# josebeo2016/SCL-Deepfake-audio-detection

Hardware: AMD Instinct MI355X
Metric: train-step utterances/sec (64000-sample clips) (higher is better)
Workload: dtype bf16

## Files before the change

include/scl_hip.h:

```cpp
#ifndef SCL_HIP_H
#define SCL_HIP_H
#include <stdint.h>
#include <stddef.h>

#ifdef __cplusplus
extern "C" {
#endif

#define SCL_OK            0
#define SCL_EINVAL       -1
#define SCL_ELAUNCH      -2
#define SCL_EUNSUPPORTED -3

int         scl_version(void);
const char* scl_last_error(void);

int scl_stream_wait_stream(void* waiter, void* signaler);

#define SCL_KID_GEMM 0
#define SCL_KID_GEMM_F32 2
#define SCL_KID_AUG  1
#define SCL_KID_MAX  8
int scl_build_flags(void);
int scl_prof_enable(int kid, int on);
int scl_prof_reserve(int kid, int n_pairs);
int scl_prof_read(int kid, int64_t* n_launches, double* total_ms, double* total_flops);
int scl_prof_read_launches(int kid, int cap, float* ms, int32_t* meta8, int64_t* n_launches);

typedef struct SclOperand {
    const void* ptr;
    int64_t bs1, bs2;
    int64_t rbstride;
    int64_t cout;
    int32_t rpb;
    int32_t ld;
    int32_t cin;
    int32_t _pad;
} SclOperand;

#define SCL_GEMM_A_T      0x00000001
#define SCL_GEMM_B_T      0x00000002
#define SCL_GEMM_C_F32    0x00000004
#define SCL_GEMM_C2_F32   0x00000008
#define SCL_GEMM_R_F32    0x00000010
#define SCL_GEMM_HAS_BIAS 0x00000020
#define SCL_GEMM_HAS_C2   0x00000040
#define SCL_GEMM_DROPOUT  0x00000080
#define SCL_GEMM_NO_DMA   0x00100000
#define SCL_GEMM_NO_BIG   0x00200000
#define SCL_GEMM_FORCE_BIG 0x04000000
#define SCL_GEMM_NO_P8    0x00400000
#define SCL_GEMM_FORCE_P8 0x00800000
#define SCL_GEMM_NO_W8    0x01000000
#define SCL_GEMM_F32X3    0x20000000
#define SCL_GEMM_FORCE_W8 0x02000000
#define SCL_GEMM_FORCE_X2 0x08000000
#define SCL_GEMM_NO_X2    0x10000000
#define SCL_GEMM_AB_F32   0x40000000
#define SCL_GEMM_C_SPLIT3 0x80000000u
#define SCL_GEMM_STAMPS   0x20000000
#define SCL_GEMM_ACT_SHIFT   8
#define SCL_GEMM_RMODE_SHIFT 12
#define SCL_GEMM_RACT_SHIFT  16

typedef struct SclGemmDesc {
    SclOperand A, B;
    void*        C;
    void*        C2;
    const void*  R;
    const float* bias;
    int64_t c_bs1, c_bs2;
    int64_t c_rbstride;
    int64_t c_split_stride;
    int64_t bias_bs2;
    int32_t c_rpb, ldc;
    int32_t M, N, K;
    int32_t nb1, nb2, splitk;
    int32_t flags;
    float    alpha;
    float    drop_p;
    uint32_t drop_seed;
    int32_t  _pad;
    float*   colsum_part;
} SclGemmDesc;

int scl_gemm_bf16(const SclGemmDesc* desc, void* stream);
int scl_gemm_bf16_group_ok(const SclGemmDesc* descs, int n);
int scl_gemm_bf16_group(const SclGemmDesc* descs, int n, void* stream);
int scl_gemm_bf16_group_tiles(const SclGemmDesc* desc);
int scl_gemm_bf16_group_part(const SclGemmDesc* descs, const int32_t* tile0, const int32_t* ntile, int n, void* stream);

int scl_gemm_uses_wide_tiles(const SclGemmDesc* desc);
int scl_gemm_colsum_rows(const SclGemmDesc* desc);

int scl_posconv_supported(int T, int K, int G, int Cg);
int scl_posconv_wgrad_supported(int T, int K, int G, int Cg);
int scl_posconv_wgrad(const void* dypad, int dy_row0, const void* xpad, float* dw, int B, int T, int K, int G, int Cg, void* stream);
int scl_posconv_mfma(const void* xpad, const void* w, float* C, const float* bias, void* c2, const float* R, int B, int T, int K, int G,
                     int Cg, int fwd, void* stream);

int scl_debug_gemm_stamps(unsigned long long* out, int nblocks);
long long scl_debug_gemm_persistent_launches(void);

int scl_gemm_splitk_finish(const SclGemmDesc* desc, const float* slabs, int nslabs, int64_t stride, void* stream);

int scl_reduce_slabs_f32(const float* slabs, float* out, int64_t n, int nslabs, int64_t stride, void* stream);
#define SCL_SLAB_MAX_JOBS 8
typedef struct SclSlabJob {
    const float* slabs;
    float*       out;
    int64_t      n, stride;
    int32_t      nslabs, _pad;
} SclSlabJob;
int scl_reduce_slabs_multi(const SclSlabJob* jobs, int njobs, void* stream);

int scl_bn_nslabs(int N);
int scl_bn_fwd(const float* x, int N, int C, const float* gamma, const float* beta, float* running_mean, float* running_var,
               long long* num_batches_tracked, int training, float momentum, float eps, int act, float* part, float* mean,
               float* rstd, float* y, void* y2, int y2_bf16, int m_W, int m_HW, int64_t m_bs, int64_t m_rs, int64_t m_cs,
               int64_t m_base, void* stream);
int scl_bn_bwd(const float* dy, const float* y, const float* x, const float* mean, const float* rstd, const float* gamma, int N, int C,
               int act, int training, float* part, float* sums, float* dgamma, float* dbeta, float* dx, int accumulate, void* stream);
int scl_pad_nhwc_f32(const float* src, int64_t rows, int C, void* dst, int dst_bf16, int m_W, int m_HW, int64_t m_bs, int64_t m_rs,
                     int64_t m_cs, int64_t m_base, void* stream);
int scl_conv_pack_weights(const float* w, float* fwd, float* bwd, int Co, int Ci, int kh, int kw, int Cp, int Cop, void* stream);
int scl_conv_wgrad_finish(const float* slabs, float* grad, int nslab, int Co, int Ci, int kh, int kw, int Cp, int accumulate, void* stream);
int scl_maxpool3_fwd(const float* x, int64_t xs_h, int64_t xs_w, int64_t xs_b, int H, int W, int B, float* y, int* idx, void* stream);
int scl_maxpool3_bwd(const float* dy, const int* idx, int H, int W, int B, float* dx, int64_t xs_h, int64_t xs_w, int64_t xs_b, void* stream);
int scl_avgpool_fwd(const float* x, int B, int R, int C, float* y, void* stream);
int scl_avgpool_bwd(const float* dy, int B, int R, int C, float* dx, void* stream);

int scl_layernorm_fwd(const void* x, int x_f32, const float* gamma, const float* beta, void* y_bf16, float* y_f32,
                      float* mean, float* rstd, int M, int C, int64_t ldx, int64_t ldy, float eps, int act, void* stream);
int scl_layernorm_bwd_nparts(int M);
int scl_layernorm_bwd(const void* dy, int dy_f32, const void* x, int x_f32, const float* mean, const float* rstd,
                      const float* gamma, const float* beta, const float* dres, float* dx_f32, void* dx_bf16,
                      float* part, int M, int C, int64_t ldx, int64_t lddy, int64_t lddx, int act, int sum_dres, int out_rpb,
                      int64_t out_rbstride, int64_t out_off, uint32_t din_seed, float din_p, uint32_t dout_seed, float dout_p, void* stream);
int scl_colreduce_f32(const float* part, float* out, int nparts, int C, int64_t pstride, int accumulate, void* stream);
#define SCL_COLREDUCE_SEGMENTS 8
#define SCL_COLSUM_MAX_GROUPS 128
#define SCL_REDUCE_MAX_JOBS 8
typedef struct SclReduceJob {
    const float* part;
    float*       out;
    float*       out2;
    int64_t      pstride;
    int32_t      nparts, C, split, _pad;
} SclReduceJob;
int scl_colreduce_multi(const SclReduceJob* jobs, int njobs, void* stream);
int scl_colreduce_seg_f32(const float* part, float* out, int nparts, int C, int64_t pstride, int accumulate, float* scratch, int* counters,
                          float* out2, int split, void* stream);
int scl_colsum_nparts(int M);
int scl_colsum_reduce_nparts(int M, int N);
int scl_colsum(const void* x, int x_f32, float* part, int M, int N, int64_t ld, void* stream);
int scl_colsum_reduce(const void* x, int x_f32, float* part, int* counters, float* out, int M, int N, int64_t ld, void* stream);

int scl_cast_f32_bf16(const float* src, void* dst, int64_t n, void* stream);
int scl_split3_f32_bf16(const float* x, int64_t rows, int K, int64_t ldx, void* out, int order, void* stream);
int scl_add_f32(const float* a, const float* b, float* out, void* out_bf16, int64_t n, void* stream);
int scl_pad_rows_bf16(const void* src, int src_f32, void* dst, const void* pre, int ract, int B, int T, int C,
                      int rows_out, int pad_before, void* stream);
int scl_col2im_bf16(const void* dcol, void* dz, int B, int Tin, int Tout, int C, int k, int s, void* stream);
int scl_conv_weight_pack(const float* w, void* wk, void* wd, int Co, int Ci, int k, int stride, void* stream);
int scl_conv_weight_unpack_grad(const float* dwk, float* dw, int Co, int Ci, int k, void* stream);
int scl_posconv_weight_pack(const float* v, const float* g, float* norm, void* wf, void* wd, int E, int Cg, int K, void* stream);
int scl_posconv_weight_bwd(const float* dwf, const float* v, const float* g, const float* norm, float* sdot_ws,
                           float* dv, float* dg, int E, int Cg, int K, void* stream);
int scl_dropout_f32(const float* x, float* y_f32, void* y_bf16, int64_t n, uint32_t seed, float p, void* stream);
int scl_dropout_rows(const void* x, void* y, int64_t R, int T, int ld, int is_f32, uint32_t seed, float p, void* stream);
int scl_meanpool_fwd(const void* h, float* emb, int B, int T, int C, void* stream);
int scl_meanpool_bwd(const float* demb, const void* pre, void* dpre, int B, int T, int C, int ract, float drop_p,
                     uint32_t seed, void* stream);
int scl_meanpool_fwd_f32(const float* h, float* emb, int B, int T, int C, void* stream);
int scl_meanpool_bwd_f32(const float* demb, const float* pre, float* dpre, int B, int T, int C, int ract, float drop_p,
                         uint32_t seed, void* stream);
int scl_utt_head_fwd(const float* emb, const float* W, const float* bias, float* logp, int B, int C, int NC, void* stream);
int scl_utt_head_bwd(const float* dlogp, const float* logp, const float* emb, const float* W, const float* demb_in,
                     float* demb, float* dW, float* db, float* ws, int B, int C, int NC, void* stream);

int scl_softmax_fwd(const float* S, void* P, int64_t R, int T, int ldS, int Tp, void* stream);
int scl_softmax_bwd(const void* P, const float* dP, void* dS, int64_t R, int T, int lddP, int Tp, void* stream);
int scl_softmax_fwd_f32(const float* S, float* P, int64_t R, int T, int ldS, int Tp, void* stream);
int scl_softmax_fwd_f32_long(const float* S, float* P, int64_t R, int T, int ldS, int Tp, void* stream);
int scl_attn_fwd(const void* qkv, void* ctx, float* lse, int B, int T, int H, int D, float scale, float drop_p, uint32_t drop_seed,
                 void* stream);
int scl_attn_fwd_fp8(const void* qkv, void* ctx, float* lse, int B, int T, int H, int D, float scale, void* stream);
int scl_attn_bwd(const void* qkv, const void* ctx, const void* dctx, const float* lse, void* dqkv, float* bias_part, int B, int T,
                 int H, int D, float scale, float drop_p, uint32_t drop_seed, void* stream);
// ... 195 lines not shown
```

scl-deepfake-audio-detection_amd/csrc/elementwise.hip:

```cpp
#include "common.h"

namespace {

__global__ void cast_f32_bf16_kernel(const float* __restrict__ src, bf16_t* __restrict__ dst, int64_t n) {
    const int64_t i0 = ((int64_t)blockIdx.x * blockDim.x + threadIdx.x) * 8;
    const int64_t step = (int64_t)gridDim.x * blockDim.x * 8;
    for (int64_t i = i0; i < n; i += step) {
        if (i + 8 <= n) {
            const float4 a = *reinterpret_cast<const float4*>(src + i);
            const float4 b = *reinterpret_cast<const float4*>(src + i + 4);
            uint4 u;
            u.x = pack_bf2(a.x, a.y); u.y = pack_bf2(a.z, a.w); u.z = pack_bf2(b.x, b.y); u.w = pack_bf2(b.z, b.w);
            *reinterpret_cast<uint4*>(dst + i) = u;
        } else {
            for (int64_t j = i; j < n; ++j) dst[j] = f2bf(src[j]);
        }
    }
}

__global__ void split3_kernel(const float* __restrict__ x, bf16_t* __restrict__ out, int64_t rows, int K, int64_t ldx, int order) {
    const int kv = K >> 3;
    const int64_t total = rows * kv;
    const int64_t step = (int64_t)gridDim.x * blockDim.x;
    for (int64_t i = (int64_t)blockIdx.x * blockDim.x + threadIdx.x; i < total; i += step) {
// ... 66 lines not shown
    const int c8n = C / 8;
    const int64_t total = (int64_t)B * Tin * c8n;
    const int64_t i0 = (int64_t)blockIdx.x * blockDim.x + threadIdx.x;
    const int64_t step = (int64_t)gridDim.x * blockDim.x;
    for (int64_t i = i0; i < total; i += step) {
        const int c = (int)(i % c8n) * 8;
        const int64_t br = i / c8n;
        const int r = (int)(br % Tin), b = (int)(br / Tin);
        float acc[8] = {0, 0, 0, 0, 0, 0, 0, 0};
        for (int j = 0; j < k; ++j) {
            const int rj = r - j;
            if (rj < 0 || (rj % s) != 0) continue;
            const int t = rj / s;
            if (t >= Tout) continue;
            const uint4 w = *reinterpret_cast<const uint4*>(dcol + (((int64_t)b * Tout + t) * k + j) * C + c);
            const uint32_t ww[4] = {w.x, w.y, w.z, w.w};
#pragma unroll
            for (int q = 0; q < 4; ++q) { acc[2 * q] += __uint_as_float(ww[q] << 16); acc[2 * q + 1] += __uint_as_float(ww[q] & 0xFFFF0000u); }
        }
        uint4 u;
        u.x = pack_bf2(acc[0], acc[1]); u.y = pack_bf2(acc[2], acc[3]); u.z = pack_bf2(acc[4], acc[5]); u.w = pack_bf2(acc[6], acc[7]);
        *reinterpret_cast<uint4*>(dz + ((int64_t)b * Tin + r) * C + c) = u;
    }
}

__global__ void conv_w_pack_kernel(const float* __restrict__ w, bf16_t* __restrict__ wk, bf16_t* __restrict__ wd, int Co, int Ci, int k,
                                   int stride) {
    const int64_t n = (int64_t)Co * Ci * k;
    for (int64_t i = (int64_t)blockIdx.x * blockDim.x + threadIdx.x; i < n; i += (int64_t)gridDim.x * blockDim.x) {
        const int ci = (int)(i % Ci);
        const int j = (int)((i / Ci) % k);
        const int co = (int)(i / ((int64_t)Ci * k));
        const bf16_t v = f2bf(w[((int64_t)co * Ci + ci) * k + j]);
        wk[i] = v;
        if (wd) {
            const int p = j % stride, q = j / stride;
            int blk = 0;
            for (int pp = 0; pp < p; ++pp) blk += (k - pp + stride - 1) / stride;
            const int nq = (k - p + stride - 1) / stride;
            blk += nq - 1 - q;
            wd[((int64_t)blk * Co + co) * Ci + ci] = v;
        }
    }
}
__global__ void conv_w_unpack_grad_kernel(const float* __restrict__ dwk, float* __restrict__ dw, int Co, int Ci, int k) {
    const int64_t n = (int64_t)Co * Ci * k;
    for (int64_t i = (int64_t)blockIdx.x * blockDim.x + threadIdx.x; i < n; i += (int64_t)gridDim.x * blockDim.x) {
        const int j = (int)(i % k);
        const int ci = (int)((i / k) % Ci);
        const int co = (int)(i / ((int64_t)Ci * k));
        dw[i] = dwk[((int64_t)co * k + j) * Ci + ci];
    }
}

__global__ __launch_bounds__(256) void posconv_norm_part_kernel(const float* __restrict__ v, float* __restrict__ part, int nrows, int K,
                                                                int rows_per_block) {
    __shared__ float red[256];
    const int j = threadIdx.x % K, rl = threadIdx.x / K, rstep = blockDim.x / K;
    const int r0 = blockIdx.x * rows_per_block, r1 = min(nrows, r0 + rows_per_block);
    float s = 0.f;
    for (int r = r0 + rl; r < r1; r += rstep) { const float t = v[(int64_t)r * K + j]; s += t * t; }
    red[threadIdx.x] = s;
    __syncthreads();
    if (threadIdx.x < K) {
        float t = 0.f;
        for (int q = 0; q < rstep; ++q) t += red[q * K + threadIdx.x];
        part[(int64_t)blockIdx.x * K + threadIdx.x] = t;
    }
}
__global__ __launch_bounds__(1024) void posconv_vec_finish_kernel(const float* __restrict__ part, float* __restrict__ out, int nparts, int K,
                                                                   int do_sqrt) {
    __shared__ float red[1024];
    const int j = threadIdx.x % K, seg = threadIdx.x / K, nseg = blockDim.x / K;
    float s = 0.f;
    for (int p = seg; p < nparts; p += nseg) s += part[(int64_t)p * K + j];
    red[threadIdx.x] = s;
    __syncthreads();
    if (threadIdx.x < K) {
        float t = 0.f;
        for (int q = 0; q < nseg; ++q) t += red[q * K + threadIdx.x];
        out[threadIdx.x] = do_sqrt ? sqrtf(t) : t;
    }
}
__global__ void posconv_pack_kernel(const float* __restrict__ v, const float* __restrict__ g, const float* __restrict__ norm,
                                    bf16_t* __restrict__ wf, bf16_t* __restrict__ wd, int E, int Cg, int K) {
    const int64_t n = (int64_t)E * Cg * K;
    for (int64_t i = (int64_t)blockIdx.x * blockDim.x + threadIdx.x; i < n; i += (int64_t)gridDim.x * blockDim.x) {
        const int j = (int)(i % K);
        const int ci = (int)((i / K) % Cg);
        const int cot = (int)(i / ((int64_t)Cg * K));
        const int grp = cot / Cg, co = cot % Cg;
        const bf16_t val = f2bf(g[j] * v[i] / norm[j]);
        wf[(((int64_t)grp * Cg + co) * K + j) * Cg + ci] = val;
        wd[(((int64_t)grp * Cg + ci) * K + (K - 1 - j)) * Cg + co] = val;
    }
}
__global__ __launch_bounds__(256) void posconv_wbwd_dot_part_kernel(const float* __restrict__ dwf, const float* __restrict__ v,
                                                                    float* __restrict__ part, int Cg, int K) {
    extern __shared__ float sm[];
    float* vl = sm;
    float* dl = sm + Cg * K;
    float* red = dl + K * (Cg + 1);
    const int cot = blockIdx.x;
    const float* vb = v + (int64_t)cot * Cg * K;
    const float* db = dwf + (int64_t)cot * K * Cg;
    for (int i = threadIdx.x; i < Cg * K; i += blockDim.x) {
        vl[i] = vb[i];
        dl[(i / Cg) * (Cg + 1) + (i % Cg)] = db[i];
    }
    __syncthreads();
    const int j = threadIdx.x % K, h = threadIdx.x / K, nh = blockDim.x / K;
    float s = 0.f;
    for (int ci = h; ci < Cg; ci += nh) s += dl[j * (Cg + 1) + ci] * vl[ci * K + j];
    red[threadIdx.x] = s;
    __syncthreads();
    if (threadIdx.x < K) {
        float t = 0.f;
        for (int q = 0; q < nh; ++q) t += red[q * K + threadIdx.x];
        part[(int64_t)cot * K + threadIdx.x] = t;
    }
}
__global__ void posconv_wbwd_apply_kernel(const float* __restrict__ dwf, const float* __restrict__ v, const float* __restrict__ g,
                                          const float* __restrict__ norm, const float* __restrict__ sdot,
                                          float* __restrict__ dv, float* __restrict__ dg, int E, int Cg, int K) {
    const int64_t n = (int64_t)E * Cg * K;
    for (int64_t i = (int64_t)blockIdx.x * blockDim.x + threadIdx.x; i < n; i += (int64_t)gridDim.x * blockDim.x) {
        const int j = (int)(i % K);
        const int ci = (int)((i / K) % Cg);
        const int cot = (int)(i / ((int64_t)Cg * K));
        const int grp = cot / Cg, co = cot % Cg;
        const float dw = dwf[(((int64_t)grp * Cg + co) * K + j) * Cg + ci];
        const float nj = norm[j];
        dv[i] = g[j] / nj * dw - g[j] * sdot[j] / (nj * nj * nj) * v[i];
        if (i < K) dg[i] = sdot[i] / norm[i];
    }
}

__device__ __forceinline__ float ld_act(const bf16_t* p, int64_t i) { return bf2f(p[i]); }
__device__ __forceinline__ float ld_act(const float* p, int64_t i) { return p[i]; }
__device__ __forceinline__ void st_act(bf16_t* p, int64_t i, float v) { p[i] = f2bf(v); }
__device__ __forceinline__ void st_act(float* p, int64_t i, float v) { p[i] = v; }
template <typename TA>
__global__ __launch_bounds__(512) void meanpool_fwd_kernel(const TA* __restrict__ h, float* __restrict__ emb, int T, int C) {
    __shared__ float red[4][128];
    const int b = blockIdx.x, g = threadIdx.x >> 7, l = threadIdx.x & 127;
    for (int c0 = 0; c0 < C; c0 += 128) {
        const int c = c0 + l;
        float s = 0.f;
        if (c < C)
            for (int t = g; t < T; t += 4) s += ld_act(h, ((int64_t)b * T + t) * C + c);
        red[g][l] = s;
        __syncthreads();
        if (g == 0 && c < C) emb[(int64_t)b * C + c] = (((red[0][l] + red[1][l]) + red[2][l]) + red[3][l]) / (float)T;
        __syncthreads();
    }
}
template <typename TA>
__global__ void meanpool_bwd_kernel(const float* __restrict__ demb, const TA* __restrict__ pre, TA* __restrict__ dpre,
                                    int B, int T, int C, int ract, float drop_p, uint32_t seed) {
    const int64_t n = (int64_t)B * T * C;
    for (int64_t i = (int64_t)blockIdx.x * blockDim.x + threadIdx.x; i < n; i += (int64_t)gridDim.x * blockDim.x) {
        const int c = (int)(i % C);
        const int b = (int)(i / ((int64_t)T * C));
        float v = demb[(int64_t)b * C + c] / (float)T;
        if (drop_p > 0.f) v *= dropout_scale(seed, (uint64_t)i, drop_p);
        v *= act_grad_f(ract, ld_act(pre, i));
        st_act(dpre, i, v);
    }
}
__global__ void utt_head_fwd_kernel(const float* __restrict__ emb, const float* __restrict__ W, const float* __restrict__ bias,
                                    float* __restrict__ logp, int B, int C, int NC) {
    const int b = blockIdx.x * (blockDim.x >> 6) + (threadIdx.x >> 6);
    const int lane = threadIdx.x & 63;
    if (b >= B) return;
    float lg[8];
    float mx = -INFINITY;
    for (int k = 0; k < NC; ++k) {
        float s = 0.f;
        for (int c = lane; c < C; c += 64) s += emb[(int64_t)b * C + c] * W[(int64_t)k * C + c];
        s = wave_sum(s) + bias[k];
        lg[k] = s;
        mx = fmaxf(mx, s);
    }
    float se = 0.f;
    for (int k = 0; k < NC; ++k) se += expf(lg[k] - mx);
    const float lse = mx + logf(se);
    if (lane == 0) for (int k = 0; k < NC; ++k) logp[(int64_t)b * NC + k] = lg[k] - lse;
}
__global__ void utt_head_bwd_kernel(const float* __restrict__ dlogp, const float* __restrict__ logp, const float* __restrict__ emb,
                                    const float* __restrict__ W, const float* __restrict__ demb_in, float* __restrict__ demb,
                                    float* __restrict__ dW, float* __restrict__ db, float* __restrict__ dlogits_ws, int B,
                                    int C, int NC) {
    for (int i = threadIdx.x; i < B; i += blockDim.x) {
        float s = 0.f;
        for (int k = 0; k < NC; ++k) s += dlogp[i * NC + k];
        for (int k = 0; k < NC; ++k) dlogits_ws[i * NC + k] = dlogp[i * NC + k] - expf(logp[i * NC + k]) * s;
    }
    __syncthreads();
    for (int i = threadIdx.x; i < B * C; i += blockDim.x) {
        const int b = i / C, c = i % C;
        float s = demb_in ? demb_in[i] : 0.f;
        for (int k = 0; k < NC; ++k) s += dlogits_ws[b * NC + k] * W[(int64_t)k * C + c];
        demb[i] = s;
    }
    for (int i = threadIdx.x; i < NC * C; i += blockDim.x) {
        const int k = i / C, c = i % C;
        float s = 0.f;
        for (int b = 0; b < B; ++b) s += dlogits_ws[b * NC + k] * emb[(int64_t)b * C + c];
        dW[i] = s;
    }
    for (int k = threadIdx.x; k < NC; k += blockDim.x) {
        float s = 0.f;
        for (int b = 0; b < B; ++b) s += dlogits_ws[b * NC + k];
        db[k] = s;
    }
}

__global__ void add_f32_kernel(const float* __restrict__ a, const float* __restrict__ b, float* __restrict__ out,
                               bf16_t* __restrict__ out_bf, int64_t n) {
    for (int64_t i = (int64_t)blockIdx.x * blockDim.x + threadIdx.x; i < n; i += (int64_t)gridDim.x * blockDim.x) {
        const float v = a[i] + (b ? b[i] : 0.f);
        if (out) out[i] = v;
        if (out_bf) out_bf[i] = f2bf(v);
    }
}

inline int grid_for(int64_t n, int per_thread = 1) {
    int64_t b = (n / per_thread + 255) / 256;
    if (b > 4096) b = 4096;
    if (b < 1) b = 1;
    return (int)b;
}

}

extern "C" int scl_cast_f32_bf16(const float* src, void* dst, int64_t n, void* stream) {
    SCL_REQUIRE(src && dst && n > 0 && ((uintptr_t)src & 15) == 0 && ((uintptr_t)dst & 15) == 0, "cast: bad args");
    hipLaunchKernelGGL(cast_f32_bf16_kernel, dim3(grid_for(n, 8)), dim3(256), 0, (hipStream_t)stream, src, (bf16_t*)dst, n);
    return scl_check_launch("scl_cast_f32_bf16");
}

extern "C" int scl_split3_f32_bf16(const float* x, int64_t rows, int K, int64_t ldx, void* out, int order, void* stream) {
    SCL_REQUIRE(x && out && rows > 0 && K >= 8 && (K & 7) == 0 && ldx >= K && (ldx & 3) == 0 && (order == 0 || order == 1), "split3: bad args (K a multiple of 8)");
    SCL_REQUIRE(((uintptr_t)x & 15) == 0 && ((uintptr_t)out & 15) == 0, "split3: operands must be 16-byte aligned");
    hipLaunchKernelGGL(split3_kernel, dim3(grid_for(rows * (K >> 3))), dim3(256), 0, (hipStream_t)stream, x, (bf16_t*)out, rows, K, ldx, order);
    return scl_check_launch("scl_split3_f32_bf16");
}

extern "C" int scl_pad_rows_bf16(const void* src, int src_f32, void* dst, const void* pre, int ract, int B, int T, int C,
                                 int rows_out, int pad_before, void* stream) {
    SCL_REQUIRE(src && dst && B > 0 && T > 0 && C > 0 && (C & 7) == 0 && rows_out >= 1, "pad_rows: bad args");
    const int64_t total = (int64_t)B * rows_out * (C / 8);
    hipStream_t s = (hipStream_t)stream;
    if (src_f32) hipLaunchKernelGGL((pad_rows_kernel<true>), dim3(grid_for(total)), dim3(256), 0, s, src, (bf16_t*)dst, (const bf16_t*)pre, B, T, C, rows_out, pad_before, ract);
    else hipLaunchKernelGGL((pad_rows_kernel<false>), dim3(grid_for(total)), dim3(256), 0, s, src, (bf16_t*)dst, (const bf16_t*)pre, B, T, C, rows_out, pad_before, ract);
    return scl_check_launch("scl_pad_rows_bf16");
}

extern "C" int scl_col2im_bf16(const void* dcol, void* dz, int B, int Tin, int Tout, int C, int k, int s, void* stream) {
    SCL_REQUIRE(dcol && dz && B > 0 && Tin > 0 && Tout > 0 && (C & 7) == 0 && k >= 1 && s >= 1, "col2im: bad args");
    const int64_t total = (int64_t)B * Tin * (C / 8);
    hipLaunchKernelGGL(col2im_kernel, dim3(grid_for(total)), dim3(256), 0, (hipStream_t)stream, (const bf16_t*)dcol, (bf16_t*)dz, B, Tin, Tout, C, k, s);
    return scl_check_launch("scl_col2im_bf16");
}

extern "C" int scl_conv_weight_pack(const float* w, void* wk, void* wd, int Co, int Ci, int k, int stride, void* stream) {
    SCL_REQUIRE(w && wk && Co > 0 && Ci > 0 && k > 0 && stride >= 1, "conv_weight_pack: bad args");
    hipLaunchKernelGGL(conv_w_pack_kernel, dim3(grid_for((int64_t)Co * Ci * k)), dim3(256), 0, (hipStream_t)stream, w, (bf16_t*)wk,
                       (bf16_t*)wd, Co, Ci, k, stride);
    return scl_check_launch("scl_conv_weight_pack");
}
extern "C" int scl_conv_weight_unpack_grad(const float* dwk, float* dw, int Co, int Ci, int k, void* stream) {
    SCL_REQUIRE(dwk && dw && Co > 0 && Ci > 0 && k > 0, "conv_weight_unpack_grad: bad args");
    hipLaunchKernelGGL(conv_w_unpack_grad_kernel, dim3(grid_for((int64_t)Co * Ci * k)), dim3(256), 0, (hipStream_t)stream, dwk, dw, Co, Ci, k);
    return scl_check_launch("scl_conv_weight_unpack_grad");
}

extern "C" int scl_posconv_weight_pack(const float* v, const float* g, float* norm, void* wf, void* wd, int E, int Cg, int K, void* stream) {
    SCL_REQUIRE(v && g && norm && wf && wd && E > 0 && Cg > 0 && K > 0 && E % Cg == 0, "posconv_weight_pack: bad args");
    hipStream_t s = (hipStream_t)stream;
    {
        SCL_REQUIRE(K <= 256 && 256 % K == 0 && E * Cg >= 2, "posconv_weight_pack: need K | 256");
        const int nrows = E * Cg;
        int nb = nrows / 2 < 256 ? nrows / 2 : 256;
        const int rpb = (nrows + nb - 1) / nb;
        float* part = reinterpret_cast<float*>(wd);
        hipLaunchKernelGGL(posconv_norm_part_kernel, dim3((nrows + rpb - 1) / rpb), dim3(256), 0, s, v, part, nrows, K, rpb);
        hipLaunchKernelGGL(posconv_vec_finish_kernel, dim3(1), dim3(1024 / K * K), 0, s, part, norm, (nrows + rpb - 1) / rpb, K, 1);
    }
    hipLaunchKernelGGL(posconv_pack_kernel, dim3(grid_for((int64_t)E * Cg * K)), dim3(256), 0, s, v, g, norm, (bf16_t*)wf, (bf16_t*)wd, E, Cg, K);
    return scl_check_launch("scl_posconv_weight_pack");
}
extern "C" int scl_posconv_weight_bwd(const float* dwf, const float* v, const float* g, const float* norm, float* sdot_ws,
                                      float* dv, float* dg, int E, int Cg, int K, void* stream) {
    SCL_REQUIRE(dwf && v && g && norm && sdot_ws && dv && dg, "posconv_weight_bwd: null pointer");
    hipStream_t s = (hipStream_t)stream;
    {
        SCL_REQUIRE(K <= 256 && 256 % K == 0, "posconv_weight_bwd: need K | 256");
        float* part = sdot_ws + K;
        const size_t lds = (size_t)(Cg * K + K * (Cg + 1) + 256) * sizeof(float);
        static bool attr_set = false;
        if (!attr_set) {
            hipFuncSetAttribute((const void*)posconv_wbwd_dot_part_kernel, hipFuncAttributeMaxDynamicSharedMemorySize, 160 * 1024);
            attr_set = true;
        }
        SCL_REQUIRE(lds <= 160 * 1024, "posconv_weight_bwd: Cg*K too large for the LDS tile");
        hipLaunchKernelGGL(posconv_wbwd_dot_part_kernel, dim3(E), dim3(256), lds, s, dwf, v, part, Cg, K);
        hipLaunchKernelGGL(posconv_vec_finish_kernel, dim3(1), dim3(1024 / K * K), 0, s, part, sdot_ws, E, K, 0);
    }
    hipLaunchKernelGGL(posconv_wbwd_apply_kernel, dim3(grid_for((int64_t)E * Cg * K)), dim3(256), 0, s, dwf, v, g, norm, sdot_ws, dv, dg, E, Cg, K);
    return scl_check_launch("scl_posconv_weight_bwd");
}

extern "C" int scl_meanpool_fwd(const void* h, float* emb, int B, int T, int C, void* stream) {
    SCL_REQUIRE(h && emb && B > 0 && T > 0 && C > 0, "meanpool_fwd: bad args");
    hipLaunchKernelGGL(meanpool_fwd_kernel<bf16_t>, dim3(B), dim3(512), 0, (hipStream_t)stream, (const bf16_t*)h, emb, T, C);
    return scl_check_launch("scl_meanpool_fwd");
}
extern "C" int scl_meanpool_fwd_f32(const float* h, float* emb, int B, int T, int C, void* stream) {
    SCL_REQUIRE(h && emb && B > 0 && T > 0 && C > 0, "meanpool_fwd_f32: bad args");
    hipLaunchKernelGGL(meanpool_fwd_kernel<float>, dim3(B), dim3(512), 0, (hipStream_t)stream, h, emb, T, C);
    return scl_check_launch("scl_meanpool_fwd_f32");
}
extern "C" int scl_meanpool_bwd(const float* demb, const void* pre, void* dpre, int B, int T, int C, int ract, float drop_p,
                                uint32_t seed, void* stream) {
    SCL_REQUIRE(demb && pre && dpre && B > 0 && T > 0 && C > 0, "meanpool_bwd: bad args");
    hipLaunchKernelGGL(meanpool_bwd_kernel<bf16_t>, dim3(grid_for((int64_t)B * T * C)), dim3(256), 0, (hipStream_t)stream, demb, (const bf16_t*)pre, (bf16_t*)dpre, B, T, C, ract, drop_p, seed);
    return scl_check_launch("scl_meanpool_bwd");
}
extern "C" int scl_meanpool_bwd_f32(const float* demb, const float* pre, float* dpre, int B, int T, int C, int ract, float drop_p,
                                    uint32_t seed, void* stream) {
    SCL_REQUIRE(demb && pre && dpre && B > 0 && T > 0 && C > 0, "meanpool_bwd_f32: bad args");
    hipLaunchKernelGGL(meanpool_bwd_kernel<float>, dim3(grid_for((int64_t)B * T * C)), dim3(256), 0, (hipStream_t)stream, demb, pre, dpre, B, T, C, ract, drop_p, seed);
    return scl_check_launch("scl_meanpool_bwd_f32");
}
extern "C" int scl_utt_head_fwd(const float* emb, const float* W, const float* bias, float* logp, int B, int C, int NC, void* stream) {
    SCL_REQUIRE(emb && W && bias && logp && B > 0 && C > 0 && NC >= 1 && NC <= 8, "utt_head_fwd: bad args");
    hipLaunchKernelGGL(utt_head_fwd_kernel, dim3((B + 3) / 4), dim3(256), 0, (hipStream_t)stream, emb, W, bias, logp, B, C, NC);
    return scl_check_launch("scl_utt_head_fwd");
}
extern "C" int scl_utt_head_bwd(const float* dlogp, const float* logp, const float* emb, const float* W, const float* demb_in,
                                float* demb, float* dW, float* db, float* ws, int B, int C, int NC, void* stream) {
    SCL_REQUIRE(dlogp && logp && emb && W && demb && dW && db && ws && B > 0 && NC <= 8, "utt_head_bwd: bad args");
    hipLaunchKernelGGL(utt_head_bwd_kernel, dim3(1), dim3(256), 0, (hipStream_t)stream, dlogp, logp, emb, W, demb_in, demb, dW, db, ws, B, C, NC);
    return scl_check_launch("scl_utt_head_bwd");
}
__global__ void dropout_f32_kernel(const float* __restrict__ x, float* __restrict__ y, bf16_t* __restrict__ y_bf, int64_t n, uint32_t seed, float p) {
    for (int64_t i = (int64_t)blockIdx.x * blockDim.x + threadIdx.x; i < n; i += (int64_t)gridDim.x * blockDim.x) {
        const float v = x[i] * dropout_scale(seed, (uint64_t)i, p);
        if (y) y[i] = v;
        if (y_bf) y_bf[i] = f2bf(v);
    }
}
extern "C" int scl_dropout_f32(const float* x, float* y_f32, void* y_bf16, int64_t n, uint32_t seed, float p, void* stream) {
    SCL_REQUIRE(x && (y_f32 || y_bf16) && n > 0 && p >= 0.f && p < 1.f, "dropout_f32: bad args");
    hipLaunchKernelGGL(dropout_f32_kernel, dim3(grid_for(n)), dim3(256), 0, (hipStream_t)stream, x, y_f32, (bf16_t*)y_bf16, n, seed, p);
    return scl_check_launch("scl_dropout_f32");
}
template <typename TX>
__global__ void dropout_rows_kernel(const TX* __restrict__ x, TX* __restrict__ y, int64_t R, int T, int ld, uint32_t seed, float p) {
    const int64_t n = R * ld;
    for (int64_t i = (int64_t)blockIdx.x * blockDim.x + threadIdx.x; i < n; i += (int64_t)gridDim.x * blockDim.x) {
        const int64_t r = i / ld;
        const int j = (int)(i - r * ld);
        float v = 0.f;
        if (j < T) {
            if constexpr (sizeof(TX) == 2) v = bf2f(x[i]); else v = x[i];
            v *= dropout_scale(seed, (uint64_t)(r * T + j), p);
        }
        if constexpr (sizeof(TX) == 2) y[i] = f2bf(v); else y[i] = v;
    }
}
extern "C" int scl_dropout_rows(const void* x, void* y, int64_t R, int T, int ld, int is_f32, uint32_t seed, float p, void* stream) {
    SCL_REQUIRE(x && y && R > 0 && T > 0 && ld >= T && p >= 0.f && p < 1.f, "dropout_rows: bad args");
    if (is_f32) hipLaunchKernelGGL(dropout_rows_kernel<float>, dim3(grid_for(R * ld)), dim3(256), 0, (hipStream_t)stream, (const float*)x, (float*)y, R, T, ld, seed, p);
    else hipLaunchKernelGGL(dropout_rows_kernel<bf16_t>, dim3(grid_for(R * ld)), dim3(256), 0, (hipStream_t)stream, (const bf16_t*)x, (bf16_t*)y, R, T, ld, seed, p);
    return scl_check_launch("scl_dropout_rows");
}
extern "C" int scl_add_f32(const float* a, const float* b, float* out, void* out_bf16, int64_t n, void* stream) {
    SCL_REQUIRE(a && (out || out_bf16) && n > 0, "add_f32: bad args");
    hipLaunchKernelGGL(add_f32_kernel, dim3(grid_for(n)), dim3(256), 0, (hipStream_t)stream, a, b, out, (bf16_t*)out_bf16, n);
    return scl_check_launch("scl_add_f32");
}
```

scl-deepfake-audio-detection_amd/csrc/gemm.hip:

```cpp
#include "gemm_common.h"

using namespace sclg;

namespace {

constexpr int BM = 128, BN = 128;

struct StageK {
    __amdgpu_buffer_rsrc_t rsrc;
    unsigned rowoff[4];
    unsigned lds_off[4];
    int kcur, kend;

    __device__ __forceinline__ void init(const OpK& o, const char* base, int row0, int rowlimit, int kbegin, int kend_, int tid) {
        rsrc = make_rsrc(base);
        const int c = tid & 7;
#pragma unroll
        for (int i = 0; i < 4; ++i) {
            const int row = (tid >> 3) + 32 * i;
            const int r = row0 + row;
            rowoff[i] = r < rowlimit ? row_off(o, (unsigned)r) : OOB;
            lds_off[i] = (unsigned)(row * 128 + ((c ^ ((row >> 1) & 7)) << 4));
        }
        kcur = kbegin + 8 * c; kend = kend_;
// ... 549 lines not shown

    f32x4 acc[2][4][4];
#pragma unroll
    for (int h = 0; h < 2; ++h)
#pragma unroll
        for (int i = 0; i < 4; ++i)
#pragma unroll
            for (int j = 0; j < 4; ++j) acc[h][i][j] = f32x4{0.f, 0.f, 0.f, 0.f};

#define P8_ISSUE_A(BUF) { la0.issue(d.A, (BUF), wave); la1.issue(d.A, (BUF) + TILE_BYTES, wave); la0.advance(); la1.advance(); }
#define P8_ISSUE_B(BUF) { lb0.issue(d.B, (BUF) + 2 * TILE_BYTES, wave); lb1.issue(d.B, (BUF) + 3 * TILE_BYTES, wave); lb0.advance(); lb1.advance(); }

    P8_ISSUE_A(smem) P8_ISSUE_B(smem) P8_ISSUE_B(smem + P8_BUF)
    asm volatile("s_waitcnt vmcnt(4)" ::: "memory");
    __builtin_amdgcn_s_barrier();
    if (wr == 1) __builtin_amdgcn_s_barrier();

    bf16x8 fa[4][2], fb0[2][2], fb1[2][2];
    for (int kt = 0; kt < nk; ++kt) {
        char* buf = smem + (kt & 1) * P8_BUF;
        char* obuf = smem + ((kt & 1) ^ 1) * P8_BUF;
        const char* tA = buf + wr * TILE_BYTES;
        const char* tB = buf + (2 + (wc >> 1)) * TILE_BYTES;
        const int nb = (wc & 1) * 4;
#pragma unroll
        for (int ks = 0; ks < 2; ++ks) {
#pragma unroll
            for (int j = 0; j < 2; ++j) fb0[j][ks] = BT ? frag_t_raw(tB, nb + j, ks, lane) : frag_k(tB, nb + j, ks, lane);
        }
        __builtin_amdgcn_sched_barrier(0);
#pragma unroll
        for (int ks = 0; ks < 2; ++ks) {
#pragma unroll
            for (int i = 0; i < 4; ++i) fa[i][ks] = AT ? frag_t_raw(tA, i, ks, lane) : frag_k(tA, i, ks, lane);
        }
        P8_ISSUE_A(obuf)
        P8_PHASE(0, 0, fb0)
#pragma unroll
        for (int ks = 0; ks < 2; ++ks) {
#pragma unroll
            for (int j = 0; j < 2; ++j) fb1[j][ks] = BT ? frag_t_raw(tB, nb + 2 + j, ks, lane) : frag_k(tB, nb + 2 + j, ks, lane);
        }
        P8_PHASE(0, 1, fb1)
#pragma unroll
        for (int ks = 0; ks < 2; ++ks) {
#pragma unroll
            for (int i = 0; i < 4; ++i) fa[i][ks] = AT ? frag_t_raw(tA, 4 + i, ks, lane) : frag_k(tA, 4 + i, ks, lane);
        }
        P8_PHASE(1, 1, fb1)
        asm volatile("s_waitcnt vmcnt(0)" ::: "memory");
        P8_ISSUE_B(buf)
        P8_PHASE(1, 0, fb0)
    }
    if (wr == 0) __builtin_amdgcn_s_barrier();
    asm volatile("s_waitcnt vmcnt(0)" ::: "memory");
    gemm_epilogue(d, acc[0], m0 + wr * 128, n0 + wc * 64, z1, z2, ksplit, lane, 0, 0);
    gemm_epilogue(d, acc[1], m0 + wr * 128 + 64, n0 + wc * 64, z1, z2, ksplit, lane, 0, 0);
}
#undef P8_PHASE
#undef P8_ISSUE_A
#undef P8_ISSUE_B

#endif

__global__ void scl_reduce_slabs_kernel(const float* __restrict__ slabs, float* __restrict__ out, int64_t n,
                                        int nslabs, int64_t stride) {
    const int64_t i0 = ((int64_t)blockIdx.x * blockDim.x + threadIdx.x) * 4;
    const int64_t step = (int64_t)gridDim.x * blockDim.x * 4;
    for (int64_t i = i0; i < n; i += step) {
        if (i + 4 <= n) {
            float4 s = *reinterpret_cast<const float4*>(slabs + i);
            for (int k = 1; k < nslabs; ++k) {
                const float4 t = *reinterpret_cast<const float4*>(slabs + k * stride + i);
                s.x += t.x; s.y += t.y; s.z += t.z; s.w += t.w;
            }
            *reinterpret_cast<float4*>(out + i) = s;
        } else {
            for (int64_t j = i; j < n; ++j) {
                float s = slabs[j];
                for (int k = 1; k < nslabs; ++k) s += slabs[k * stride + j];
                out[j] = s;
            }
        }
    }
}

}

namespace sclg {
void make_magic(unsigned dv, unsigned* magic, unsigned* shift) {
    unsigned l = 0;
    while ((1ull << l) < dv) ++l;
    *shift = l;
    *magic = (unsigned)((((1ull << l) - dv) << 32) / dv + 1);
}

bool fill_operand(const SclOperand& o, const char* name, long long rows, long long contig, OpK* k, int esz) {
    const int vec = 16 / esz;
    if (!o.ptr || ((uintptr_t)o.ptr & 15)) { scl_set_error("gemm: %s ptr null or not 16B aligned", name); return false; }
    if (o.rpb < 1 || o.cin < vec) { scl_set_error("gemm: %s rpb/cin invalid", name); return false; }
    if ((o.ld % vec) || (o.rbstride % vec) || (o.cout % vec) || (o.bs1 % vec) || (o.bs2 % vec) || (o.cin != 0x7fffffff && (o.cin % vec))) {
        scl_set_error("gemm: %s strides must be multiples of %d elements", name, vec); return false;
    }
    const long long rq = (rows - 1) / o.rpb, rr = o.rpb == 0x7fffffff ? rows - 1 : (long long)o.rpb - 1;
    const long long cq = o.cin == 0x7fffffff ? 0 : (contig - 1) / o.cin;
    const long long cr = o.cin == 0x7fffffff ? contig - 1 : (long long)o.cin - 1;
    const long long maxoff = rq * o.rbstride + (rr < rows - 1 ? rr : rows - 1) * (long long)o.ld + cq * o.cout + cr + vec;
    if (maxoff < 0 || maxoff * esz >= (1ll << 32) - 32 || rows >= (1ll << 31)) {
        scl_set_error("gemm: %s extent exceeds 32-bit byte offsets (%lld elements)", name, maxoff); return false;
    }
    k->ptr = o.ptr; k->bs1 = o.bs1 * esz; k->bs2 = o.bs2 * esz;
    k->rb_bytes = (unsigned)(o.rbstride * esz); k->ld_bytes = (unsigned)o.ld * (unsigned)esz; k->cout_bytes = (unsigned)(o.cout * esz);
    k->rpb = (unsigned)o.rpb; make_magic((unsigned)o.rpb, &k->rpb_magic, &k->rpb_shift);
    k->cin = (unsigned)o.cin; make_magic((unsigned)o.cin, &k->cin_magic, &k->cin_mshift);
    k->esz_shift = esz == 4 ? 2u : 1u;
    return true;
}
}

namespace {

bool gemm_pick_w8(const GemmK& k, bool at, bool bt, const SclGemmDesc& d, long long zdim, W8Plan* plan) {
    const int w8_env = 1;
    if (d.flags & (SCL_GEMM_NO_W8 | SCL_GEMM_FORCE_P8 | SCL_GEMM_FORCE_BIG | SCL_GEMM_NO_DMA)) return false;
    const bool a_whole = at ? (d.M % 8 == 0) : (d.K % 8 == 0);
    const bool b_whole = bt ? (d.N % 8 == 0) : (d.K % 8 == 0);
    static const int ncu_env = [] { const char* e = getenv("SCL_GEMM_CUS"); const int v = e ? atoi(e) : 256; return v >= 32 && v <= 256 ? v : 256; }();
    if (!a_whole || !b_whole || !scl_gemm_w8_plan(k, at, bt, d, zdim, ncu_env, plan)) return false;
    const long long need = at ? 128 : 160;
    return (d.flags & SCL_GEMM_FORCE_W8) || (w8_env && d.N >= 192 && plan->tiles * zdim >= need);
}

#ifdef SCL_EXPERIMENTS
bool gemm_pick_x2(const GemmK& k, bool at, bool bt, const SclGemmDesc& d, long long zdim, W8Plan* plan) {
    static const int x2_env = [] { const char* e = getenv("SCL_GEMM_X2"); return e ? atoi(e) : 0; }();
    if (d.flags & (SCL_GEMM_NO_X2 | SCL_GEMM_FORCE_W8 | SCL_GEMM_FORCE_P8 | SCL_GEMM_FORCE_BIG | SCL_GEMM_NO_DMA)) return false;
    if (!(d.flags & SCL_GEMM_FORCE_X2) && x2_env == 0) return false;
    const bool a_whole = at ? (d.M % 8 == 0) : (d.K % 8 == 0);
    const bool b_whole = bt ? (d.N % 8 == 0) : (d.K % 8 == 0);
    static const int ncu_env = [] { const char* e = getenv("SCL_GEMM_CUS"); const int v = e ? atoi(e) : 256; return v >= 32 && v <= 256 ? v : 256; }();
    if (!a_whole || !b_whole || !scl_gemm_x2_plan(k, at, bt, d, zdim, ncu_env, plan)) return false;
    if ((d.flags & SCL_GEMM_FORCE_X2) || x2_env == 2) return true;
    return !at && d.N >= 128 && plan->tiles * zdim >= 248;
}

#else
bool gemm_pick_x2(const GemmK&, bool, bool, const SclGemmDesc&, long long, W8Plan*) { return false; }
#endif
}

extern "C" int scl_gemm_uses_wide_tiles(const SclGemmDesc* dp) {
    if (!dp || dp->M <= 0 || dp->N <= 0 || dp->K <= 0 || dp->nb1 < 1 || dp->nb2 < 1 || dp->splitk < 1) return 0;
    GemmK k; W8Plan plan;
    const bool at = dp->flags & SCL_GEMM_A_T, bt = dp->flags & SCL_GEMM_B_T;
    const long long zdim = (long long)dp->nb1 * dp->nb2 * dp->splitk;
    if (gemm_pick_x2(k, at, bt, *dp, zdim, &plan)) return 3;
    return gemm_pick_w8(k, at, bt, *dp, zdim, &plan) ? (plan.variant == 2 ? 4 : 1 + plan.variant) : 0;
}

static int gemm_colsum_rows(const SclGemmDesc& d) {
    if (d.M <= 0 || d.N <= 0 || d.K <= 0 || d.nb1 != 1 || d.nb2 != 1 || d.splitk != 1 || (d.N & 7) || (d.ldc & 7) || (d.flags & SCL_GEMM_AB_F32)) return 0;
    GemmK k; W8Plan plan;
    const bool at = d.flags & SCL_GEMM_A_T, bt = d.flags & SCL_GEMM_B_T;
    const bool a_whole = at ? (d.M % 8 == 0) : (d.K % 8 == 0), b_whole = bt ? (d.N % 8 == 0) : (d.K % 8 == 0);
    SclGemmDesc dq = d;
    if (!dq.colsum_part) dq.colsum_part = reinterpret_cast<float*>(16);
// ... 243 lines not shown
    float v[4] = {0.f, 0.f, 0.f, 0.f};
    const bool full = col + 4 <= d.N && !(d.N & 3) && !(stride & 3);
    for (int s = 0; s < nslabs; ++s, p += stride) {
        if (full) {
            const float4 t = *reinterpret_cast<const float4*>(p);
            v[0] += t.x; v[1] += t.y; v[2] += t.z; v[3] += t.w;
        } else {
            for (int i = 0; i < 4; ++i) if (col + i < d.N) v[i] += p[i];
        }
    }
    const unsigned q = udiv_magic((unsigned)row, d.c_magic, d.c_shift);
    const long long off = (long long)q * d.c_rbstride + (long long)((unsigned)row - q * d.c_rpb) * d.ldc + col;
    const float* bias = (flags & SCL_GEMM_HAS_BIAS) ? d.bias : nullptr;
    if (full && d.vec_ok) {
        const bool c_f32 = flags & SCL_GEMM_C_F32, c2_f32 = flags & SCL_GEMM_C2_F32, r_f32 = flags & SCL_GEMM_R_F32;
        const int act = (flags >> SCL_GEMM_ACT_SHIFT) & 0xF, rmode = (flags >> SCL_GEMM_RMODE_SHIFT) & 0xF, ract = (flags >> SCL_GEMM_RACT_SHIFT) & 0xF;
        if (bias) {
            const float4 bb = *reinterpret_cast<const float4*>(bias + col);
            v[0] += bb.x; v[1] += bb.y; v[2] += bb.z; v[3] += bb.w;
        }
        float c2v[4] = {v[0], v[1], v[2], v[3]};
        if (act == 5) { gelu_both_f(v[0], v[0], c2v[0]); gelu_both_f(v[1], v[1], c2v[1]); gelu_both_f(v[2], v[2], c2v[2]); gelu_both_f(v[3], v[3], c2v[3]); }
        if (flags & SCL_GEMM_HAS_C2) {
            if (c2_f32) *reinterpret_cast<float4*>(reinterpret_cast<float*>(d.C2) + off) = make_float4(c2v[0], c2v[1], c2v[2], c2v[3]);
            else *reinterpret_cast<uint2*>(reinterpret_cast<bf16_t*>(d.C2) + off) = make_uint2(pack_bf2(c2v[0], c2v[1]), pack_bf2(c2v[2], c2v[3]));
        }
        if (act && act != 5) { v[0] = act_f(act, v[0]); v[1] = act_f(act, v[1]); v[2] = act_f(act, v[2]); v[3] = act_f(act, v[3]); }
        float r[4] = {0.f, 0.f, 0.f, 0.f};
        if (rmode) {
            if (r_f32) {
                const float4 t = *reinterpret_cast<const float4*>(reinterpret_cast<const float*>(d.R) + off);
                r[0] = t.x; r[1] = t.y; r[2] = t.z; r[3] = t.w;
            } else {
                const uint2 t = *reinterpret_cast<const uint2*>(reinterpret_cast<const bf16_t*>(d.R) + off);
                r[0] = __uint_as_float(t.x << 16); r[1] = __uint_as_float(t.x & 0xFFFF0000u);
                r[2] = __uint_as_float(t.y << 16); r[3] = __uint_as_float(t.y & 0xFFFF0000u);
            }
        }
#pragma unroll
        for (int i = 0; i < 4; ++i) {
            if (rmode == 2) v[i] *= act_grad_f(ract, r[i]);
            if (flags & SCL_GEMM_DROPOUT) v[i] *= dropout_scale(d.drop_seed, (uint64_t)(off + i), d.drop_p);
            if (rmode == 1) v[i] += r[i];
        }
        if (c_f32) *reinterpret_cast<float4*>(reinterpret_cast<float*>(d.C) + off) = make_float4(v[0], v[1], v[2], v[3]);
        else *reinterpret_cast<uint2*>(reinterpret_cast<bf16_t*>(d.C) + off) = make_uint2(pack_bf2(v[0], v[1]), pack_bf2(v[2], v[3]));
    } else {
        const EpiArgs ea = {d.C, d.C2, d.R, d.N, d.flags, d.drop_seed, d.drop_p};
        for (int i = 0; i < 4; ++i) epi_scalar(ea, v[i], off + i, col + i, bias);
    }
}

extern "C" int scl_gemm_splitk_finish(const SclGemmDesc* dp, const float* slabs, int nslabs, int64_t stride, void* stream) {
    SCL_REQUIRE(dp && slabs && nslabs >= 1 && stride >= 0, "gemm finish: bad args");
    const SclGemmDesc& d = *dp;
    SCL_REQUIRE(d.M > 0 && d.N > 0 && d.nb1 == 1 && d.nb2 == 1, "gemm finish: one un-batched [M, N] problem");
    SCL_REQUIRE(d.C && d.c_rpb >= 1, "gemm finish: C null or c_rpb < 1");
    const int rmode = (d.flags >> SCL_GEMM_RMODE_SHIFT) & 0xF;
    SCL_REQUIRE(rmode == 0 || d.R, "gemm finish: RMODE set but R is null");
    SCL_REQUIRE(!(d.flags & SCL_GEMM_HAS_C2) || d.C2, "gemm finish: HAS_C2 set but C2 is null");
    SCL_REQUIRE(!(d.flags & SCL_GEMM_HAS_BIAS) || d.bias, "gemm finish: HAS_BIAS set but bias is null");
    SCL_REQUIRE(((uintptr_t)slabs & 15) == 0, "gemm finish: slabs must be 16-byte aligned");
    GemmK k;
    k.C = d.C; k.C2 = d.C2; k.R = d.R; k.bias = d.bias; k.colsum = nullptr;
    k.c_bs1 = 0; k.c_bs2 = 0; k.c_rbstride = d.c_rbstride; k.c_split_stride = 0; k.bias_bs2 = 0;
    k.c_rpb = (unsigned)d.c_rpb; make_magic((unsigned)d.c_rpb, &k.c_magic, &k.c_shift);
    k.ldc = d.ldc; k.M = d.M; k.N = d.N; k.K = d.K; k.nb2 = 1; k.splitk = 1; k.flags = d.flags;
    k.alpha = 1.0f; k.drop_p = d.drop_p; k.drop_seed = d.drop_seed; k.group_m = 8; k.tile_m = 0; k.debug = 0;
    auto al = [](const void* p, int bytes) { return p == nullptr || ((uintptr_t)p & (bytes - 1)) == 0; };
    k.vec_ok = !(d.ldc & 3) && !(d.c_rbstride & 3) && al(d.C, (d.flags & SCL_GEMM_C_F32) ? 16 : 8) && al(d.C2, (d.flags & SCL_GEMM_C2_F32) ? 16 : 8) &&
               al(d.R, (d.flags & SCL_GEMM_R_F32) ? 16 : 8) && al(d.bias, 16);
    const long long n = (long long)d.M * ((d.N + 3) / 4);
    hipLaunchKernelGGL(scl_gemm_finish_kernel, dim3((unsigned)((n + 255) / 256)), dim3(256), 0, (hipStream_t)stream, k, slabs, nslabs, (long long)stride);
    return scl_check_launch("scl_gemm_splitk_finish");
}

extern "C" int scl_reduce_slabs_f32(const float* slabs, float* out, int64_t n, int nslabs, int64_t stride, void* stream) {
    SCL_REQUIRE(slabs && out && n > 0 && nslabs >= 1, "reduce_slabs: bad args");
    SCL_REQUIRE(((uintptr_t)slabs & 15) == 0 && ((uintptr_t)out & 15) == 0 && (stride & 3) == 0, "reduce_slabs: alignment");
    int blocks = (int)((n / 4 + 255) / 256); if (blocks > 2048) blocks = 2048; if (blocks < 1) blocks = 1;
    hipLaunchKernelGGL(scl_reduce_slabs_kernel, dim3(blocks), dim3(256), 0, (hipStream_t)stream, slabs, out, n, nslabs, stride);
    return scl_check_launch("scl_reduce_slabs_f32");
}
```

scl-deepfake-audio-detection_amd/csrc/gemm_w8.hip:

```cpp
#include "gemm_common.h"
#include "gemm_w8_epi.h"

using namespace sclg;

__device__ unsigned long long scl_gemm_stamps[4096 * 8];

namespace {

__device__ __forceinline__ void w8_stamp(const GemmK& d, int slot, int lane, int wave) {
    if ((d.flags & SCL_GEMM_STAMPS) && wave == 0 && lane == 0 && blockIdx.x < 4096 && blockIdx.z == 0) {
        scl_gemm_stamps[blockIdx.x * 8 + 2 * slot] = __builtin_amdgcn_s_memrealtime();
        scl_gemm_stamps[blockIdx.x * 8 + 2 * slot + 1] = __builtin_amdgcn_s_memtime();
    }
}

constexpr int W8_BN = 256;
constexpr int W8_OPB = 2 * TILE_BYTES;
constexpr int W8_NA = 3, W8_NB = 2;
constexpr int W8_LDS = (W8_NA + W8_NB) * W8_OPB;

struct W8K {
    __amdgpu_buffer_rsrc_t rsrc;
    unsigned voff[4];
    __device__ __forceinline__ void init(const OpK& o, const char* base, int row0, int rowlimit, int lane, int wave) {
        rsrc = make_rsrc(base);
#pragma unroll
        for (int i = 0; i < 4; ++i) {
            const int row = 8 * (wave * 4 + i) + (lane >> 3);
            const int r = row0 + row;
            const int kc = (lane & 7) ^ ((row >> 1) & 7);
            voff[i] = r < rowlimit ? row_off(o, (unsigned)r) + (unsigned)(kc << 4) : OOB;
        }
    }
    template <int I0>
    __device__ __forceinline__ void issue2(char* img, int wave, unsigned soff, bool live) const {
#pragma unroll
        for (int i = I0; i < I0 + 2; ++i) {
            const unsigned off = live ? voff[i] : OOB;
            __builtin_amdgcn_raw_ptr_buffer_load_lds(rsrc, (lds_void*)(img + (wave * 4 + i) * 1024), 16, off, soff, 0, 0);
        }
    }
    __device__ __forceinline__ void issue1(char* img, int wave, unsigned soff, bool live, int i) const {
        const unsigned off = live ? voff[i] : OOB;
        __builtin_amdgcn_raw_ptr_buffer_load_lds(rsrc, (lds_void*)(img + (wave * 4 + i) * 1024), 16, off, soff, 0, 0);
    }
    __device__ __forceinline__ static unsigned kstep(const OpK& o) { return o.cin == 64 ? o.cout_bytes : 128u; }
    __device__ __forceinline__ void rows(const OpK&, int, int, int) {}
    __device__ __forceinline__ void set_batched(bool) {}
    __device__ __forceinline__ unsigned step(const OpK& o) const { return kstep(o); }
};
struct W8T {
    __amdgpu_buffer_rsrc_t rsrc;
    unsigned voff[4];
    int col0_, collimit_;
    bool batched;
    __device__ __forceinline__ void set_batched(bool b) { batched = b; }
    __device__ __forceinline__ void init(const OpK& o, const char* base, int col0, int collimit, int lane, int wave) {
        rsrc = make_rsrc(base);
        col0_ = col0; collimit_ = collimit;
        const int s16 = lane & 15;
#pragma unroll
        for (int i = 0; i < 4; ++i) {
            const int p = wave * 4 + i;
            const int kr = 4 * (p & 15) + (lane >> 4);
            const int sw = (kr & 3) | (((kr >> 3) & 1) << 2);
            const int col = col0 + (p >> 4) * 128 + 8 * ((((s16 >> 1) ^ sw) << 1) | (s16 & 1));
            voff[i] = col < collimit ? (unsigned)kr * o.ld_bytes + col_off(o, (unsigned)col) : OOB;
        }
    }
    __device__ __forceinline__ void rows(const OpK& o, int krow, int lane, int wave) {
        if (!batched) return;
        const int s16 = lane & 15;
#pragma unroll
        for (int i = 0; i < 4; ++i) {
            const int p = wave * 4 + i;
            const int kr = 4 * (p & 15) + (lane >> 4);
            const int sw = (kr & 3) | (((kr >> 3) & 1) << 2);
            const int col = col0_ + (p >> 4) * 128 + 8 * ((((s16 >> 1) ^ sw) << 1) | (s16 & 1));
            voff[i] = col < collimit_ ? row_off(o, (unsigned)(krow + kr)) + col_off(o, (unsigned)col) : OOB;
        }
    }
    template <int I0>
    __device__ __forceinline__ void issue2(char* img, int wave, unsigned soff, bool live) const {
#pragma unroll
        for (int i = I0; i < I0 + 2; ++i) {
            const unsigned off = live ? voff[i] : OOB;
            __builtin_amdgcn_raw_ptr_buffer_load_lds(rsrc, (lds_void*)(img + (wave * 4 + i) * 1024), 16, off, soff, 0, 0);
        }
    }
    __device__ __forceinline__ void issue1(char* img, int wave, unsigned soff, bool live, int i) const {
        const unsigned off = live ? voff[i] : OOB;
        __builtin_amdgcn_raw_ptr_buffer_load_lds(rsrc, (lds_void*)(img + (wave * 4 + i) * 1024), 16, off, soff, 0, 0);
    }
    __device__ __forceinline__ static unsigned kstep(const OpK& o) { return 64u * o.ld_bytes; }
    __device__ __forceinline__ unsigned step(const OpK& o) const { return batched ? 0u : kstep(o); }
};
template <bool T> struct W8Sel { typedef W8K type; };
template <> struct W8Sel<true> { typedef W8T type; };

template <bool T>
__device__ __forceinline__ bf16x8 w8_frag(const char* img, int gb, int ks, int lane) {
    if (T) return frag_t_raw(img + (gb >> 3) * TILE_BYTES, gb & 7, ks, lane);
    return frag_k(img, gb, ks, lane);
}

#define W8_MFMA_PHASE(MH, NH, FBSEL, NI)                                                                   \
    asm volatile("s_waitcnt lgkmcnt(0)" ::: "memory");                                                     \
    __builtin_amdgcn_sched_barrier(0);                                                                     \
    __builtin_amdgcn_s_barrier();                                                                          \
    __builtin_amdgcn_sched_barrier(0);                                                                     \
    __builtin_amdgcn_s_setprio(1);                                                                         \
    _Pragma("unroll") for (int ks = 0; ks < 2; ++ks)                                                       \
        _Pragma("unroll") for (int i = 0; i < (NI); ++i)                                                   \
            _Pragma("unroll") for (int j = 0; j < 2; ++j)                                                  \
                acc[MH][i][2 * (NH) + j] = __builtin_amdgcn_mfma_f32_16x16x32_bf16(FBSEL[j][ks], fa[i][ks], acc[MH][i][2 * (NH) + j], 0, 0, 0); \
    __builtin_amdgcn_s_setprio(0);                                                                         \
    __builtin_amdgcn_sched_barrier(0);                                                                     \
    __builtin_amdgcn_s_barrier();

template <bool AT, bool BT, int NH>
__device__ __forceinline__ void w8_body(const GemmK& d, char* smem, typename W8Sel<AT>::type& la, typename W8Sel<BT>::type& lb,
                                        int nk, unsigned soffA, unsigned soffB, int ab, int m0, int n0, int mlimit,
                                        int z1, int z2, int ksplit, int lane, int wave, int wc, int krow0) {
    const unsigned stepA = la.step(d.A), stepB = lb.step(d.B);
    f32x4 acc[2][4][4];
#pragma unroll
    for (int h = 0; h < 2; ++h)
#pragma unroll
        for (int i = 0; i < 4; ++i)
#pragma unroll
            for (int j = 0; j < 4; ++j) acc[h][i][j] = f32x4{0.f, 0.f, 0.f, 0.f};

    bf16x8 fa[4][2], fb0[2][2], fb1[2][2];
    const int nbk = wc * 4;
    char* const bimg = smem + W8_NA * W8_OPB;
    char *a_cur = smem, *a_nxt = smem + W8_OPB, *a_fill = smem + 2 * W8_OPB;
    for (int kt = 0; kt < nk; ++kt) {
        const char* tA = a_cur;
        char* tB = bimg + (kt & 1) * W8_OPB;
#ifdef W8_FAKE_AB
        const bool live2 = false;
#else
        const bool live2 = kt + 2 < nk;
#endif
        soffA += stepA; soffB += stepB;
#pragma unroll
        for (int ks = 0; ks < 2; ++ks) {
#pragma unroll
            for (int j = 0; j < 2; ++j) fb0[j][ks] = w8_frag<BT>(tB, nbk + j, ks, lane);
        }
        __builtin_amdgcn_sched_barrier(0);
#pragma unroll
        for (int ks = 0; ks < 2; ++ks) {
#pragma unroll
            for (int i = 0; i < 4; ++i) fa[i][ks] = w8_frag<AT>(tA, ab + i, ks, lane);
        }
        la.rows(d.A, krow0 + (kt + 2) * BK, lane, wave);
        la.template issue2<0>(a_fill, wave, soffA, live2);
        W8_MFMA_PHASE(0, 0, fb0, 4)
#pragma unroll
        for (int ks = 0; ks < 2; ++ks) {
#pragma unroll
            for (int j = 0; j < 2; ++j) fb1[j][ks] = w8_frag<BT>(tB, nbk + 2 + j, ks, lane);
        }
        la.template issue2<2>(a_fill, wave, soffA, live2);
        W8_MFMA_PHASE(0, 1, fb1, 4)
#pragma unroll
        for (int ks = 0; ks < 2; ++ks) {
#pragma unroll
            for (int i = 0; i < NH; ++i) fa[i][ks] = w8_frag<AT>(tA, ab + 4 + i, ks, lane);
        }
        lb.rows(d.B, krow0 + (kt + 2) * BK, lane, wave);
        lb.template issue2<0>(tB, wave, soffB, live2);
        W8_MFMA_PHASE(1, 1, fb1, NH)
        lb.template issue2<2>(tB, wave, soffB, live2);
        asm volatile("s_waitcnt vmcnt(8)" ::: "memory");
        W8_MFMA_PHASE(1, 0, fb0, NH)
        char* t = a_cur; a_cur = a_nxt; a_nxt = a_fill; a_fill = t;
    }
    if ((wave >> 2) == 0) __builtin_amdgcn_s_barrier();
    asm volatile("s_waitcnt vmcnt(0)" ::: "memory");
    __builtin_amdgcn_s_barrier();
    w8_stamp(d, 2, lane, wave);
    {
        const long long cbase = z1 * d.c_bs1 + z2 * d.c_bs2 + (long long)ksplit * d.c_split_stride;
        const float* bias = (d.flags & SCL_GEMM_HAS_BIAS) ? d.bias + z2 * d.bias_bs2 : nullptr;
        char* wlds = smem + wave * 16384;
        char* wextra = smem + 8 * 16384 + wave * 4096;
        float* cs0 = d.colsum ? d.colsum + ((long long)(m0 / d.tile_m) * 4 + (wave >> 2) * 2) * d.N : nullptr;
        w8_epilogue_pass<4, 0>(d, acc[0], 4, wlds, wextra, m0 + ab * 16, n0 + wc * 64, mlimit, cbase, bias, lane, cs0);
        w8_epilogue_pass<4, 0>(d, acc[1], NH, wlds, wextra, m0 + (ab + 4) * 16, n0 + wc * 64, mlimit, cbase, bias, lane, cs0 ? cs0 + d.N : nullptr);
    }
    if (d.flags & SCL_GEMM_STAMPS) {
        asm volatile("s_waitcnt vmcnt(0)" ::: "memory");
        w8_stamp(d, 3, lane, wave);
    }
}

template <bool AT, bool BT, int RB0, int RB1>
__global__ __launch_bounds__(512, 2) void scl_gemm_w8_kernel(const GemmK d) {
    extern __shared__ __attribute__((aligned(16))) char smem[];
    const int tid = threadIdx.x, lane = tid & 63;
    const int wave = __builtin_amdgcn_readfirstlane(tid >> 6);
    const int wr = wave >> 2, wc = wave & 3;
    w8_stamp(d, 0, lane, wave);
    const int tiles_m = (d.M + d.tile_m - 1) / d.tile_m, tiles_n = (d.N + W8_BN - 1) / W8_BN;
    int tm, tn;
    tile_coords(blockIdx.x, gridDim.x, tiles_m, tiles_n, tm, tn, d.group_m);
    const int m0 = tm * d.tile_m, n0 = tn * W8_BN;
    const int mlimit = min(d.M, m0 + d.tile_m);
    int z = blockIdx.z;
    const int ksplit = __builtin_amdgcn_readfirstlane(z % d.splitk); z /= d.splitk;
    const int z1 = __builtin_amdgcn_readfirstlane(z / d.nb2), z2 = z - z1 * d.nb2;
    const int nk_total = d.K / BK;
    const int nk_per = __builtin_amdgcn_readfirstlane((nk_total + d.splitk - 1) / d.splitk);
    const int kt0 = ksplit * nk_per;
    const int nk = max(0, min(nk_per, nk_total - kt0));
    const char* Ab = reinterpret_cast<const char*>(d.A.ptr) + z1 * d.A.bs1 + z2 * d.A.bs2;
    const char* Bb = reinterpret_cast<const char*>(d.B.ptr) + z1 * d.B.bs1 + z2 * d.B.bs2;

    typename W8Sel<AT>::type la;
    typename W8Sel<BT>::type lb;
    la.init(d.A, Ab, m0, mlimit, lane, wave);
    lb.init(d.B, Bb, n0, d.N, lane, wave);
    la.set_batched(AT && (d.debug & 4));
    lb.set_batched(BT && (d.debug & 8));
    const unsigned stepA = la.step(d.A), stepB = lb.step(d.B);
    unsigned soffA = (unsigned)kt0 * stepA, soffB = (unsigned)kt0 * stepB;
    const int krow0 = kt0 * BK;

    la.rows(d.A, krow0, lane, wave); lb.rows(d.B, krow0, lane, wave);
    la.template issue2<0>(smem, wave, soffA, nk > 0); la.template issue2<2>(smem, wave, soffA, nk > 0);
    lb.template issue2<0>(smem + W8_NA * W8_OPB, wave, soffB, nk > 0); lb.template issue2<2>(smem + W8_NA * W8_OPB, wave, soffB, nk > 0);
    soffA += stepA; soffB += stepB;
    la.rows(d.A, krow0 + BK, lane, wave); lb.rows(d.B, krow0 + BK, lane, wave);
    la.template issue2<0>(smem + W8_OPB, wave, soffA, nk > 1); la.template issue2<2>(smem + W8_OPB, wave, soffA, nk > 1);
    lb.template issue2<0>(smem + (W8_NA + 1) * W8_OPB, wave, soffB, nk > 1); lb.template issue2<2>(smem + (W8_NA + 1) * W8_OPB, wave, soffB, nk > 1);
    asm volatile("s_waitcnt vmcnt(8)" ::: "memory");
    w8_stamp(d, 1, lane, wave);
    __builtin_amdgcn_s_barrier();
    if (wr == 1) __builtin_amdgcn_s_barrier();

    if (RB0 == RB1) {
        w8_body<AT, BT, RB0 - 4>(d, smem, la, lb, nk, soffA, soffB, wr * RB0, m0, n0, mlimit, z1, z2, ksplit, lane, wave, wc, krow0);
    } else if (wr == 0) {
        w8_body<AT, BT, RB0 - 4>(d, smem, la, lb, nk, soffA, soffB, 0, m0, n0, mlimit, z1, z2, ksplit, lane, wave, wc, krow0);
    } else {
        w8_body<AT, BT, RB1 - 4>(d, smem, la, lb, nk, soffA, soffB, RB0, m0, n0, mlimit, z1, z2, ksplit, lane, wave, wc, krow0);
    }
}

template <int OFF>
__device__ __forceinline__ bf16x8 lds_b128_raw(unsigned addr) {
    bf16x8 v;
    asm volatile("ds_read_b128 %0, %1 offset:%2" : "=v"(v) : "v"(addr), "n"(OFF) : "memory");
    return v;
}
template <bool AT, bool BT, int RBW>
struct W8SRead {
    static constexpr bool RAW = AT || BT;
    static __device__ __forceinline__ unsigned kaddr(const char* img, int gb, int ks, int lane) {
        const int row = gb * 16 + (lane & 15);
        const int c = 4 * ks + (lane >> 4);
        return (unsigned)(uintptr_t)(lds_void*)(img + row * 128 + ((c ^ ((row >> 1) & 7)) << 4));
    }
    template <int R, int REND>
    static __device__ __forceinline__ void step(bf16x8 (&FA)[RBW], bf16x8 (&FB)[4], const char* TA, const char* TB, unsigned ka, unsigned kb,
                                                int ab, int nbk, int ks, int lane) {
        if constexpr (R < REND) {
            if constexpr (R == 0 || (R > RBW)) {
                constexpr int j = R == 0 ? 0 : R - RBW;
                if constexpr (BT) FB[j] = frag_t_raw(TB + ((nbk + j) >> 3) * TILE_BYTES, (nbk + j) & 7, ks, lane);
                else if constexpr (RAW) FB[j] = lds_b128_raw<j * 2048>(kb);
                else FB[j] = frag_k(TB, nbk + j, ks, lane);
            } else {
                constexpr int i = R - 1;
                if constexpr (AT) FA[i] = frag_t_raw(TA + ((ab + i) >> 3) * TILE_BYTES, (ab + i) & 7, ks, lane);
                else if constexpr (RAW) FA[i] = lds_b128_raw<i * 2048>(ka);
                else FA[i] = frag_k(TA, ab + i, ks, lane);
            }
            if (RAW) __builtin_amdgcn_sched_barrier(0);
            step<R + 1, REND>(FA, FB, TA, TB, ka, kb, ab, nbk, ks, lane);
        }
    }
    template <int R0, int R1, bool ORDERED>
    static __device__ __forceinline__ void go(bf16x8 (&FA)[RBW], bf16x8 (&FB)[4], const char* TA, const char* TB, int ab, int nbk, int ks, int lane) {
        if constexpr (R0 < R1) {
            unsigned ka = 0, kb = 0;
            if constexpr (RAW && !AT) ka = kaddr(TA, ab, ks, lane);
            if constexpr (RAW && !BT) kb = kaddr(TB, nbk, ks, lane);
            if constexpr (ORDERED && !RAW) {
                step<R0, R0 + 1>(FA, FB, TA, TB, ka, kb, ab, nbk, ks, lane);
                __builtin_amdgcn_sched_barrier(0);
                go<R0 + 1, R1, true>(FA, FB, TA, TB, ab, nbk, ks, lane);
            } else {
                step<R0, R1>(FA, FB, TA, TB, ka, kb, ab, nbk, ks, lane);
            }
        }
    }
};

template <bool AT, bool BT, int RBW>
__device__ __forceinline__ void w8s_body(const GemmK& d, char* smem, const typename W8Sel<AT>::type& la, const typename W8Sel<BT>::type& lb,
                                         int nk, unsigned soffA, unsigned soffB, int ab, int m0, int n0, int mlimit,
                                         int z1, int z2, int ksplit, int lane, int wave, int wc) {
    const unsigned stepA = W8Sel<AT>::type::kstep(d.A), stepB = W8Sel<BT>::type::kstep(d.B);
    f32x4 acc[RBW][4];
#pragma unroll
    for (int i = 0; i < RBW; ++i)
#pragma unroll
        for (int j = 0; j < 4; ++j) acc[i][j] = f32x4{0.f, 0.f, 0.f, 0.f};
    bf16x8 fa0[RBW], fa1[RBW], fb0[4], fb1[4];
    const int nbk = wc * 4;
    char* const bimg = smem + W8_NA * W8_OPB;
    char *a_cur = smem, *a_nxt = smem + W8_OPB, *a_fill = smem + 2 * W8_OPB;
    constexpr int NRD = RBW + 4, OPA = AT ? 2 : 1, OPB = BT ? 2 : 1;
    constexpr int RQ0 = NRD < 4 ? NRD : 4, RQ1 = NRD < 8 ? NRD : 8, RQ2 = NRD;
    typedef W8SRead<AT, BT, RBW> RD;
    auto ops_upto = [](int n) constexpr { return (n > 0 ? OPB : 0) + (n > 1 ? (n - 1 < RBW ? n - 1 : RBW) * OPA : 0) + (n > RBW + 1 ? (n - RBW - 1) * OPB : 0); };
    lds_wait_upto(0);
    __builtin_amdgcn_sched_barrier(0);
    RD::template go<0, NRD, true>(fa0, fb0, a_cur, bimg, ab, nbk, 0, lane);
    for (int kt = 0; kt < nk; ++kt) {
        char* tB = bimg + (kt & 1) * W8_OPB;
        const bool live2 = kt + 2 < nk;
#ifdef W8S_FAKE_A
        const bool live2a = false;
#else
        const bool live2a = live2;
#endif
#ifdef W8S_FAKE_B
        const bool live2b = false;
#else
        const bool live2b = live2;
#endif
        soffA += stepA; soffB += stepB;
#define W8S_Q_FIRST(j, R0, R1)                                                                                               \
        RD::template go<R0, R1, false>(fa1, fb1, a_cur, tB, ab, nbk, 1, lane);                                               \
        __builtin_amdgcn_sched_barrier(0);                                                                                   \
        lds_wait_upto((3 - (j)) * OPB + ops_upto(R1));                                                                       \
        __builtin_amdgcn_sched_barrier(0);                                                                                   \
        _Pragma("unroll") for (int i = 0; i < RBW; ++i)                                                                      \
            acc[i][j] = __builtin_amdgcn_mfma_f32_16x16x32_bf16(fb0[j], fa0[i], acc[i][j], 0, 0, 0);                         \
        __builtin_amdgcn_sched_barrier(0);                                                                                   \
        la.issue1(a_fill, wave, soffA, live2a, j);                                                                           \
        __builtin_amdgcn_sched_barrier(0);
        W8S_Q_FIRST(0, 0, RQ0) W8S_Q_FIRST(1, RQ0, RQ1) W8S_Q_FIRST(2, RQ1, RQ2) W8S_Q_FIRST(3, RQ2, NRD)
#undef W8S_Q_FIRST
        lds_wait_upto(0);
        asm volatile("s_waitcnt vmcnt(4)" ::: "memory");
        __builtin_amdgcn_sched_barrier(0);
        __builtin_amdgcn_s_barrier();
        __builtin_amdgcn_sched_barrier(0);
        const char* tBn = bimg + ((kt & 1) ^ 1) * W8_OPB;
#define W8S_B_ISSUE(j) if ((j) < 2) { lb.issue1(tB, wave, soffB, live2b, 2 * (j)); lb.issue1(tB, wave, soffB, live2b, 2 * (j) + 1); }
#define W8S_Q_SECOND(j, R0, R1)                                                                                              \
        RD::template go<R0, R1, false>(fa0, fb0, a_nxt, tBn, ab, nbk, 0, lane);                                              \
        __builtin_amdgcn_sched_barrier(0);                                                                                   \
        _Pragma("unroll") for (int i = 0; i < RBW; ++i)                                                                      \
            acc[i][j] = __builtin_amdgcn_mfma_f32_16x16x32_bf16(fb1[j], fa1[i], acc[i][j], 0, 0, 0);                         \
        __builtin_amdgcn_sched_barrier(0);                                                                                   \
        W8S_B_ISSUE(j)                                                                                                       \
        __builtin_amdgcn_sched_barrier(0);
        W8S_Q_SECOND(0, 0, RQ0) W8S_Q_SECOND(1, RQ0, RQ1) W8S_Q_SECOND(2, RQ1, RQ2) W8S_Q_SECOND(3, RQ2, NRD)
#undef W8S_Q_SECOND
#undef W8S_B_ISSUE
        char* t = a_cur; a_cur = a_nxt; a_nxt = a_fill; a_fill = t;
    }
    asm volatile("s_waitcnt vmcnt(0)" ::: "memory");
    asm volatile("s_waitcnt lgkmcnt(0)" ::: "memory");
    __builtin_amdgcn_s_barrier();
    w8_stamp(d, 2, lane, wave);
    {
        const long long cbase = z1 * d.c_bs1 + z2 * d.c_bs2 + (long long)ksplit * d.c_split_stride;
        const float* bias = (d.flags & SCL_GEMM_HAS_BIAS) ? d.bias + z2 * d.bias_bs2 : nullptr;
        char* wlds = smem + wave * 16384;
        char* wextra = smem + 8 * 16384 + wave * 4096;
        float* cs0 = d.colsum ? d.colsum + ((long long)(m0 / d.tile_m) * 4 + (wave >> 2) * 2) * d.N : nullptr;
        if constexpr (RBW >= 4) {
            f32x4 (&alo)[4][4] = *reinterpret_cast<f32x4 (*)[4][4]>(&acc[0]);
            w8_epilogue_pass<4, ((RBW < 8 && !AT) ? 0x1E : 0)>(d, alo, 4, wlds, wextra, m0 + ab * 16, n0 + wc * 64, mlimit, cbase, bias, lane, cs0);
        } else {
            f32x4 lo[4][4];
#pragma unroll
            for (int i = 0; i < 4; ++i)
#pragma unroll
                for (int j = 0; j < 4; ++j) lo[i][j] = (i < RBW) ? acc[(i < RBW) ? i : 0][j] : f32x4{0.f, 0.f, 0.f, 0.f};
            w8_epilogue_pass<4, ((RBW < 8 && !AT) ? 0x1E : 0)>(d, lo, RBW, wlds, wextra, m0 + ab * 16, n0 + wc * 64, mlimit, cbase, bias, lane, cs0);
        }
        if (RBW > 4) {
            f32x4 hi[4][4];
#pragma unroll
            for (int i = 0; i < 4; ++i)
#pragma unroll
                for (int j = 0; j < 4; ++j) hi[i][j] = (4 + i < RBW) ? acc[(4 + i < RBW) ? 4 + i : 0][j] : f32x4{0.f, 0.f, 0.f, 0.f};
            w8_epilogue_pass<4, ((RBW < 8 && !AT) ? 0x1E : 0)>(d, hi, RBW - 4, wlds, wextra, m0 + (ab + 4) * 16, n0 + wc * 64, mlimit, cbase, bias, lane, cs0 ? cs0 + d.N : nullptr);
        }
    }
    if (d.flags & SCL_GEMM_STAMPS) {
        asm volatile("s_waitcnt vmcnt(0)" ::: "memory");
        w8_stamp(d, 3, lane, wave);
    }
}

template <bool AT, bool BT, int RB0, int RB1, bool SEQ = false>
__device__ __forceinline__ void w8s_tile(const GemmK& d, char* smem, const int bid, const int nblk, const int bz) {
    const int tid = threadIdx.x, lane = tid & 63;
    const int wave = __builtin_amdgcn_readfirstlane(tid >> 6);
    const int wr = wave >> 2, wc = wave & 3;
    w8_stamp(d, 0, lane, wave);
#ifdef SCL_EXPERIMENTS
    if ((d.debug >> 8) && (bid & 1) && bid < 256 && bz == 0) {
        for (int i = 0; i < (d.debug >> 8); ++i) __builtin_amdgcn_s_sleep(127);
    }
#endif
    const int tiles_m = (d.M + d.tile_m - 1) / d.tile_m, tiles_n = (d.N + W8_BN - 1) / W8_BN;
    int tm, tn;
    tile_coords<SEQ>(bid, nblk, tiles_m, tiles_n, tm, tn, d.group_m);
    const int m0 = tm * d.tile_m, n0 = tn * W8_BN;
    const int mlimit = min(d.M, m0 + d.tile_m);
    int z = bz;
    const int ksplit = __builtin_amdgcn_readfirstlane(z % d.splitk); z /= d.splitk;
    const int z1 = __builtin_amdgcn_readfirstlane(z / d.nb2), z2 = z - z1 * d.nb2;
    const int nk_total = d.K / BK;
    const int nk_per = __builtin_amdgcn_readfirstlane((nk_total + d.splitk - 1) / d.splitk);
    const int kt0 = ksplit * nk_per;
    const int nk = max(0, min(nk_per, nk_total - kt0));
    const char* Ab = reinterpret_cast<const char*>(d.A.ptr) + z1 * d.A.bs1 + z2 * d.A.bs2;
    const char* Bb = reinterpret_cast<const char*>(d.B.ptr) + z1 * d.B.bs1 + z2 * d.B.bs2;

    typename W8Sel<AT>::type la;
    typename W8Sel<BT>::type lb;
    la.init(d.A, Ab, m0, mlimit, lane, wave);
    lb.init(d.B, Bb, n0, d.N, lane, wave);
    la.set_batched(false); lb.set_batched(false);
    const unsigned stepA = W8Sel<AT>::type::kstep(d.A), stepB = W8Sel<BT>::type::kstep(d.B);
    unsigned soffA = (unsigned)kt0 * stepA, soffB = (unsigned)kt0 * stepB;
    la.template issue2<0>(smem, wave, soffA, nk > 0); la.template issue2<2>(smem, wave, soffA, nk > 0);
    lb.template issue2<0>(smem + W8_NA * W8_OPB, wave, soffB, nk > 0); lb.template issue2<2>(smem + W8_NA * W8_OPB, wave, soffB, nk > 0);
    soffA += stepA; soffB += stepB;
    la.template issue2<0>(smem + W8_OPB, wave, soffA, nk > 1); la.template issue2<2>(smem + W8_OPB, wave, soffA, nk > 1);
    lb.template issue2<0>(smem + (W8_NA + 1) * W8_OPB, wave, soffB, nk > 1); lb.template issue2<2>(smem + (W8_NA + 1) * W8_OPB, wave, soffB, nk > 1);
    asm volatile("s_waitcnt vmcnt(8)" ::: "memory");
    w8_stamp(d, 1, lane, wave);
    __builtin_amdgcn_s_barrier();
    if (RB0 == RB1) {
        w8s_body<AT, BT, RB0>(d, smem, la, lb, nk, soffA, soffB, wr * RB0, m0, n0, mlimit, z1, z2, ksplit, lane, wave, wc);
    } else if (wr == 0) {
        w8s_body<AT, BT, RB0>(d, smem, la, lb, nk, soffA, soffB, 0, m0, n0, mlimit, z1, z2, ksplit, lane, wave, wc);
    } else {
        w8s_body<AT, BT, RB1>(d, smem, la, lb, nk, soffA, soffB, RB0, m0, n0, mlimit, z1, z2, ksplit, lane, wave, wc);
    }
}

template <bool AT, bool BT, int RB0, int RB1>
__global__ __launch_bounds__(512, 2) void scl_gemm_w8s_kernel(const GemmK d) {
    extern __shared__ __attribute__((aligned(16))) char smem[];
    w8s_tile<AT, BT, RB0, RB1>(d, smem, blockIdx.x, gridDim.x, blockIdx.z);
}

struct GemmGroupK {
    GemmK k[W8_GROUP_MAX];
    int first[W8_GROUP_MAX + 1];
    int tile0[W8_GROUP_MAX];
    int ntiles[W8_GROUP_MAX];
    int n;
    int xcd_major;
};
typedef const __attribute__((address_space(4))) GemmGroupK* W8GArg;
template <bool AT, bool BT, int RB0, int RB1>
__global__ __launch_bounds__(512, 2) void scl_gemm_w8s_group_kernel(const GemmGroupK g) {
    extern __shared__ __attribute__((aligned(16))) char smem[];
    W8GArg gp = (W8GArg)__builtin_amdgcn_kernarg_segment_ptr();
    const int total = g.first[W8_GROUP_MAX];
    const int x = blockIdx.x & 7, idx = blockIdx.x >> 3, q = total >> 3, r = total & 7;
#ifdef SCL_EXPERIMENTS
    const int pos = (g.xcd_major ? ((x < r ? x * (q + 1) : r * (q + 1) + (x - r) * q) + idx) : (int)blockIdx.x);
#else
    const int pos = (x < r ? x * (q + 1) : r * (q + 1) + (x - r) * q) + idx;
#endif
    int mem = 0;
#pragma unroll
    for (int i = 1; i < W8_GROUP_MAX; ++i) mem += (i < g.n && pos >= g.first[i]) ? 1 : 0;
    mem = __builtin_amdgcn_readfirstlane(mem);
    const int t = __builtin_amdgcn_readfirstlane(pos - gp->first[mem] + gp->tile0[mem]);
#ifdef SCL_EXPERIMENTS
    if (!g.xcd_major) { w8s_tile<AT, BT, RB0, RB1, false>(*(const GemmK*)&gp->k[mem], smem, t, gp->ntiles[mem], 0); return; }
#endif
    w8s_tile<AT, BT, RB0, RB1, true>(*(const GemmK*)&gp->k[mem], smem, t, gp->ntiles[mem], 0);
}

#ifdef SCL_EXPERIMENTS
typedef const __attribute__((address_space(4))) GemmK* W8KArg;
__device__ __forceinline__ const GemmK* w8p_args(W8KArg p) {
    asm volatile("" : "+s"(p));
    return (const GemmK*)p;
}
template <bool AT, bool BT, int RBW>
__device__ __forceinline__ void w8p_body(const GemmK& d, W8KArg kp, char* smem, const char* Ab, const char* Bb, int ab, int tiles_m, int tiles_n,
                                         int lane, int wave, int wc) {
    typedef typename W8Sel<AT>::type LA;
    typedef typename W8Sel<BT>::type LB;
    const unsigned stepA = LA::kstep(d.A), stepB = LB::kstep(d.B);
    const int nk = d.K / BK;
    const int ntiles = tiles_m * tiles_n, G = gridDim.x;
    const int nbk = wc * 4;
    char* const bimg = smem + W8_NA * W8_OPB;
    char *a_cur = smem, *a_nxt = smem + W8_OPB, *a_fill = smem + 2 * W8_OPB;
    int bpar = 0;
    int v = blockIdx.x, tm, tn;
    tile_coords(v, ntiles, tiles_m, tiles_n, tm, tn, d.group_m);
    const int tile_m = d.tile_m, Mrows = d.M, group_m = d.group_m;
    int m0 = tm * tile_m, n0 = tn * W8_BN, mlimit = min(Mrows, m0 + tile_m);
    LA la;
    LB lb;
    la.init(d.A, Ab, m0, mlimit, lane, wave);
    lb.init(d.B, Bb, n0, d.N, lane, wave);
    la.set_batched(false); lb.set_batched(false);
    la.template issue2<0>(a_cur, wave, 0u, true); la.template issue2<2>(a_cur, wave, 0u, true);
    lb.template issue2<0>(bimg, wave, 0u, true); lb.template issue2<2>(bimg, wave, 0u, true);
    la.template issue2<0>(a_nxt, wave, stepA, true); la.template issue2<2>(a_nxt, wave, stepA, true);
    lb.template issue2<0>(bimg + W8_OPB, wave, stepB, true); lb.template issue2<2>(bimg + W8_OPB, wave, stepB, true);
    asm volatile("s_waitcnt vmcnt(8)" ::: "memory");
    __builtin_amdgcn_s_barrier();
#define W8S_READ(FA, FB, TA, TB, KS)                                                        \
    _Pragma("unroll") for (int j = 0; j < 4; ++j) FB[j] = w8_frag<BT>(TB, nbk + j, KS, lane); \
    _Pragma("unroll") for (int i = 0; i < RBW; ++i) FA[i] = w8_frag<AT>(TA, ab + i, KS, lane);
#define W8S_MFMA(FA, FB)                                                                    \
    _Pragma("unroll") for (int i = 0; i < RBW; ++i)                                         \
        _Pragma("unroll") for (int j = 0; j < 4; ++j)                                       \
            acc[i][j] = __builtin_amdgcn_mfma_f32_16x16x32_bf16(FB[j], FA[i], acc[i][j], 0, 0, 0);
    for (;;) {
        f32x4 acc[RBW][4];
#pragma unroll
        for (int i = 0; i < RBW; ++i)
#pragma unroll
            for (int j = 0; j < 4; ++j) acc[i][j] = f32x4{0.f, 0.f, 0.f, 0.f};
        bf16x8 fa0[RBW], fa1[RBW], fb0[4], fb1[4];
        const int vn = v + G;
        const bool has_next = vn < ntiles;
        int m0n = 0, n0n = 0, mlimn = 0;
        if (has_next) {
            tile_coords(vn, ntiles, tiles_m, tiles_n, tm, tn, group_m);
            m0n = tm * tile_m; n0n = tn * W8_BN; mlimn = min(Mrows, m0n + tile_m);
        }
        unsigned soffA = stepA, soffB = stepB;
        W8S_READ(fa0, fb0, a_cur, bimg + bpar * W8_OPB, 0)
        for (int kt = 0; kt < nk; ++kt) {
            char* tB = bimg + ((kt + bpar) & 1) * W8_OPB;
            const bool hand = kt + 2 == nk;
            const bool live2 = kt + 2 < nk || (hand && has_next);
            soffA += stepA; soffB += stepB;
            asm volatile("s_waitcnt lgkmcnt(0)" ::: "memory");
            __builtin_amdgcn_sched_barrier(0);
            W8S_READ(fa1, fb1, a_cur, tB, 1)
            __builtin_amdgcn_sched_barrier(0);
            W8S_MFMA(fa0, fb0)
            __builtin_amdgcn_sched_barrier(0);
            if (hand && has_next) {
                const GemmK* dh = w8p_args(kp);
                la.init(dh->A, reinterpret_cast<const char*>(dh->A.ptr), m0n, mlimn, lane, wave);
            }
            {
                const unsigned sa = hand ? 0u : soffA;
                la.template issue2<0>(a_fill, wave, sa, live2); la.template issue2<2>(a_fill, wave, sa, live2);
            }
            asm volatile("s_waitcnt lgkmcnt(0)" ::: "memory");
            asm volatile("s_waitcnt vmcnt(4)" ::: "memory");
            __builtin_amdgcn_sched_barrier(0);
            __builtin_amdgcn_s_barrier();
            __builtin_amdgcn_sched_barrier(0);
            if (hand && has_next) {
// ... 140 lines not shown
    const bool b_ok = bt ? (flat_rows(d.B, d.K) || (tt && d.B.rpb >= 1)) : (d.B.cin == 0x7fffffff || d.B.cin == 64 || d.B.cin >= d.K);
    if (!a_ok || !b_ok || (d.K % BK) != 0) return false;
    const long long tiles_n = (d.N + W8_BN - 1) / W8_BN;
    long long best = -1;
    const char* e43 = getenv("SCL_W8_TILE112");
    const char* epp = getenv("SCL_W8_MODE");
    const bool v43_env = !e43 || atoi(e43) != 0, pingpong_env = epp && *epp && atoi(epp) == 0;
    const bool v43_ok = v43_env && !pingpong_env && !at && zdim == 1 && !d.colsum_part && !(d.flags & SCL_GEMM_STAMPS);
    for (int v = 0; v < (v43_ok ? 3 : 2); ++v) {
        const int bm = v == 0 ? 208 : (v == 1 ? 256 : 112);
        const long long ntm = (d.M + bm - 1) / bm;
        const long long rounds = (ntm * tiles_n * zdim + ncu - 1) / ncu;
        const long long cost = rounds * (bm + W8_BN);
        if (best < 0 || cost < best) {
            best = cost;
            plan->variant = v; plan->tiles_m = (int)ntm; plan->tile_m = (int)((d.M + ntm - 1) / ntm);
            plan->tiles = ntm * tiles_n; plan->cost = cost; plan->ncu = ncu;
        }
    }
    return true;
}

bool scl_gemm_w8_group_member_ok(const GemmK& k, bool at, bool bt, const SclGemmDesc& d) {
    if (!at || !bt || d.nb1 != 1 || d.nb2 != 1 || d.splitk != 1 || (d.K % BK) != 0 || d.K / BK < 3) return false;
    if ((long long)d.A.rpb < (long long)d.K || (long long)d.B.rpb < (long long)d.K) return false;
    if ((d.M % 8) || (d.N % 8) || !k.vec_ok) return false;
    const int plain = SCL_GEMM_A_T | SCL_GEMM_B_T | SCL_GEMM_C_F32;
    return (d.flags & ~(SCL_GEMM_NO_DMA | SCL_GEMM_NO_W8)) == plain && !d.colsum_part;
}

int scl_gemm_w8_group_tiles(const GemmK& k) { return ((k.M + 255) / 256) * ((k.N + W8_BN - 1) / W8_BN); }

int scl_gemm_w8_group_launch(GemmK* ks, int n, const int* tile0, const int* ntile, hipStream_t s) {
    GemmGroupK g = GemmGroupK();
    int total = 0;
    for (int i = 0; i < n; ++i) {
        GemmK& k = ks[i];
        const int ntm = (k.M + 255) / 256;
        k.tile_m = (k.M + ntm - 1) / ntm;
        k.debug = 0;
        g.k[i] = k;
        g.first[i] = total;
        g.ntiles[i] = scl_gemm_w8_group_tiles(k);
        g.tile0[i] = tile0 ? tile0[i] : 0;
        total += ntile ? ntile[i] : g.ntiles[i];
    }
    for (int i = n; i <= W8_GROUP_MAX; ++i) g.first[i] = total;
    g.n = n;
#ifdef SCL_EXPERIMENTS
    static const int xcd_major = [] { const char* e = getenv("SCL_WGRAD_XCD_MAJOR"); return e ? atoi(e) : 1; }();
    g.xcd_major = xcd_major;
#else
    g.xcd_major = 1;
#endif
    static bool attr_set = false;
    if (!attr_set) {
        (void)hipFuncSetAttribute((const void*)scl_gemm_w8s_group_kernel<true, true, 8, 8>, hipFuncAttributeMaxDynamicSharedMemorySize, W8_LDS);
        attr_set = true;
    }
    SCL_LAUNCH((scl_gemm_w8s_group_kernel<true, true, 8, 8>), dim3((unsigned)total), dim3(512), W8_LDS, s, g);
    return 0;
}

static long long w8p_launches = 0;
long long scl_gemm_w8p_launches() { return w8p_launches; }

int scl_gemm_read_stamps(unsigned long long* out, int nblocks) {
    return hipMemcpyFromSymbol(out, HIP_SYMBOL(scl_gemm_stamps), sizeof(unsigned long long) * 8 * (size_t)nblocks) == hipSuccess ? 0 : -1;
}

int scl_gemm_w8_launch(GemmK& k, bool at, bool bt, const W8Plan& plan, long long zdim, hipStream_t s) {
    k.tile_m = plan.tile_m;
    k.debug = 0;
    {
        const long long nb1 = zdim / ((long long)k.nb2 * k.splitk);
        const long long rows = k.M - 1, rpb = (long long)k.c_rpb;
        const long long maxoff = (nb1 - 1) * k.c_bs1 + ((long long)k.nb2 - 1) * k.c_bs2 + (rows / rpb) * k.c_rbstride + (rows % rpb) * k.ldc + k.N;
        if (maxoff * ((k.flags & SCL_GEMM_R_F32) ? 4 : 2) >= 0xFFFFFF00ll) k.debug |= 2;
    }
    const dim3 grid((unsigned)plan.tiles, 1, (unsigned)zdim);
    const char* me = getenv("SCL_W8_MODE");
    int mode = (me && *me) ? atoi(me) : 1;
    if (at && bt) {
        if ((long long)k.A.rpb < (long long)k.K) { k.debug |= 4; mode = 0; }
        if ((long long)k.B.rpb < (long long)k.K) { k.debug |= 8; mode = 0; }
    }
    {
        static const bool epi_generic = [] { const char* e = getenv("SCL_W8_EPI_GENERIC"); return e && atoi(e) != 0; }();
        if (epi_generic) k.debug |= 16;
    }
    dim3 g = grid;
#ifdef SCL_EXPERIMENTS
    {
        const char* sg = getenv("SCL_W8_STAGGER");
        const int stg = sg ? atoi(sg) : 0;
        if (stg > 0 && plan.tiles > 256 && zdim == 1) k.debug |= (stg & 0xFF) << 8;
    }
    const char* pe = getenv("SCL_GEMM_PERSIST");
    const int pv = pe ? atoi(pe) : 0;
    if (mode == 1 && pv > 0 && !(at && bt) && zdim == 1 && k.splitk == 1 && k.K / BK >= 3 && !(k.flags & SCL_GEMM_STAMPS)) {
        const long long ncu = plan.ncu >= 8 ? plan.ncu : 256;
        const long long rounds = (plan.tiles + ncu - 1) / ncu;
        long long G = pv >= 8 ? (pv & ~7) : ((((plan.tiles + rounds - 1) / rounds) + 7) & ~7ll);
        if (G > (ncu & ~7ll) && pv < 8) G = ncu & ~7ll;
        if (plan.variant == 0 && (pv >= 8 || rounds >= 2) && G >= 8 && G < plan.tiles) { mode = 2; g = dim3((unsigned)G, 1, 1); ++w8p_launches; }
    }
#endif
    if (plan.variant == 2) w8_launch_43(k, bt, g, s);
    else if (plan.variant == 0) w8_launch_rb<7, 6>(k, at, bt, g, s, mode);
    else w8_launch_rb<8, 8>(k, at, bt, g, s, mode);
    return 0;
}

}
```

scl-deepfake-audio-detection_amd/encoder.py:

```python
import contextlib
import os

import torch

from . import ops
from .lib import ACT_GELU, ACT_GELU_DC2, FLAT, RACT_STORED, SclError
from .ops import Op

FUSED_BIAS_GRAD = True
WGRAD_SMALL_SPLIT = True
BATCH_REDUCE = True
BATCH_SLABS = True
WGRAD_GROUP = os.environ.get("SCL_WGRAD_GROUP", "1") != "0"
WGRAD_CARRY = os.environ.get("SCL_WGRAD_CARRY", "1") != "0"
WGRAD_GROUP_MIN_KSTEPS = 16
POSCONV_MFMA = True
GELU_DC2 = True
ATTN_FP8 = os.environ.get("SCL_ATTN_FP8", "0") == "1"
ATTN_LONG = os.environ.get("SCL_ATTN_LONG", "0") == "1"
MAT_ATTN_MAX_T = 512
F32_ATTN_CHUNK_BYTES = 1 << 30
SCORE_X3PLANES = os.environ.get("SCL_SCORE_X3PLANES", "1") != "0"
CONV_WGRAD_WIDE = True

# ... 168 lines not shown
            d["S"] = f32(B * H * T * Tp)
            d["P"] = [bf(B * H * T * Tp + 1024) for _ in range(cfg.layers)]
        d["ctx"] = [bfz(Mp, E) for _ in range(cfg.layers)]
        d["x1"] = [f32(M * E) for _ in range(cfg.layers)]
        d["m2"], d["r2"] = [f32(M) for _ in range(cfg.layers)], [f32(M) for _ in range(cfg.layers)]
        d["h2"] = [bfz(Mp, E) for _ in range(cfg.layers)]
        d["f"] = [bf(M * Fd) for _ in range(cfg.layers)]
        d["a"] = [bfz(Mp, Fd) for _ in range(cfg.layers)]
        d["out"], d["omean"], d["orstd"] = bf(M * E), f32(M), f32(M)
        d["dx_rot"] = [(f32(M * E), bfz(Mp, E, slack)) for _ in range(5)]
        d["d_f"] = [bfz(Mp, Fd, slack), bfz(Mp, Fd, slack)]
        d["d_h"] = bf(M * E + slack)
        d["d_ctx"] = bf(M * E + slack)
        d["dqkv"] = [bfz(Mp, 3 * E, slack), bfz(Mp, 3 * E, slack)]
        d["dS"] = None if (d["fused_attn"] or d["long_attn"]) else bf(B * H * T * Tp + 1024)
        d["dcpad"] = bf(B * (T + K) * E + slack)
        d["dz"] = [bf(B * t * C + slack) for t in Ts]
        d["dyp"], d["dyp_geom"] = [None], [None]
        for i in range(1, len(Ts)):
            k, s, Tin, Tout = cfg.conv_kernels[i], cfg.conv_strides[i], Ts[i - 1], Ts[i]
            Q = (k - 1) // s
            Qe = max(0, max((Tin - 1 - p) // s for p in range(s)) - (Tout - 1))
            Rp = Q + Tout + Qe
            d["dyp"].append(torch.zeros(B * Rp * C + slack, dtype=torch.bfloat16, device=dev))
            d["dyp_geom"].append((Q, Rp))
        nln = max(ops.layernorm_bwd_nparts(B * t) for t in Ts)
        d["ln_part"] = f32(nln * 3 * max(C, E))
        d["ln_part2"] = f32(nln * 3 * E)
        ncs = max(ops.colsum_nparts(B * (max(Ts[1:] + [T + K]) + 4)), 1) + 1
        d["cs_part"] = f32(ncs * max(3 * E, Fd, C))
        d["qkv_bias_part"] = f32(B * 3 * E)
        d["cs_fused"] = f32(4 * (M // 200 + 2) * Fd)
        d["conv0_ws"] = f32(ops.conv0_bwd_nparts(B, L, cfg.conv_kernels[0], cfg.conv_strides[0]) * C * (cfg.conv_kernels[0] + 3))
        d["conv0_stats"] = f32(B * Ts[0] * 2)
        d["slab"] = None
        kmax = max(cfg.conv_kernels[1:]) if len(cfg.conv_kernels) > 1 else 1
        d["dwk"] = f32(C * kmax * C)
        d["dwf"] = f32(E * (E // cfg.pos_groups) * K)
        self._bufs[key] = d
        return d

    SITE_IN, SITE_ENC, SITE_ATTN, SITE_1, SITE_2, SITE_3 = 1, 2, 3, 4, 5, 6

    @staticmethod
    def site_seed(step_seed, layer, site):
        x = (int(step_seed) * 0x9E3779B1 + (layer + 1) * 0x85EBCA77 + site * 0xC2B2AE3D) & 0xFFFFFFFF
        x ^= x >> 15
        x = (x * 0x2C1B3C6D) & 0xFFFFFFFF
        x ^= x >> 12
        return x & 0x7FFFFFFF

    def drop_probs(self, training):
        c = self.cfg
        if not training:
            return 0.0, 0.0, 0.0, 0.0
        return float(c.dropout), float(c.attention_dropout), float(c.activation_dropout), float(c.dropout_input)

    @staticmethod
    def _slot(slots, handle, pos, layer, site):
        if handle is not None:
            slots.append((handle, pos, layer, site))

    def apply_seeds(self, slots, step_seed):
        for handle, pos, layer, site in slots:
            sd = self.site_seed(step_seed, layer, site)
            if pos is None:
                handle.drop_seed = sd
            else:
                handle[1][pos] = sd

    @contextlib.contextmanager
    def _side(self):
        if self.wstream is None:
            yield
            return
        ops.stream_wait(self.wstream, torch.cuda.current_stream())
        with torch.cuda.stream(self.wstream):
            yield

    def _join_side(self):
        if self.wstream is not None:
            ops.stream_wait(torch.cuda.current_stream(), self.wstream)

    def _wgrad(self, d, A, B_, out, Mo, No, Kr, slot=None, **kw):
        ksteps = (Kr + 63) // 64
        if WGRAD_GROUP and slot is not None and not kw and Kr % 64 == 0 and ksteps >= WGRAD_GROUP_MIN_KSTEPS:
            d.setdefault("wgrad_group", []).append((A, B_, out, Mo, No, Kr, slot))
            return
        tiles = ((Mo + 127) // 128) * ((No + 127) // 128) * kw.get("nb2", 1)
        sk = _splitk(tiles, ksteps)
        t256 = ((Mo + 255) // 256) * ((No + 255) // 256) * kw.get("nb2", 1)
        if t256 >= 32 or ((WGRAD_SMALL_SPLIT or (CONV_WGRAD_WIDE and ksteps >= 700)) and t256 >= 12):
            skw = max(1, min(8 if t256 >= 32 else (21 if ksteps >= 700 else 16), (256 + t256 // 2) // t256, ksteps // 8))
            if ops.gemm_wide_kind(A, B_, out, Mo, No, Kr, a_t=True, b_t=True, splitk=skw, c_split_stride=out.numel() if skw > 1 else 0, **kw):
                sk = skw
        if sk == 1:
            ops.gemm(A, B_, out, Mo, No, Kr, a_t=True, b_t=True, **kw)
            return
        n = out.numel()
        if BATCH_SLABS and slot is not None:
            bufs = d.setdefault("slab_slots", {})
            if slot not in bufs or bufs[slot].numel() < sk * n:
                d.setdefault("slabs_keep", []).append(bufs.get(slot))
                bufs[slot] = torch.empty(sk * n, dtype=torch.float32, device=self.dev)
            ops.gemm(A, B_, bufs[slot], Mo, No, Kr, a_t=True, b_t=True, splitk=sk, c_split_stride=n, **kw)
            d.setdefault("slab_jobs", []).append((bufs[slot], out, n, sk, n))
            return
        if d["slab"] is None or d["slab"].numel() < sk * n:
            d.setdefault("slabs_keep", []).append(d["slab"])
            d["slab"] = torch.empty(sk * n, dtype=torch.float32, device=self.dev)
        ops.gemm(A, B_, d["slab"], Mo, No, Kr, a_t=True, b_t=True, splitk=sk, c_split_stride=n, **kw)
        ops.reduce_slabs(d["slab"], out, n, sk, n)

    def _flush_slabs(self, d, final=True):
        group = d.get("wgrad_group")
        pend = d.setdefault("wgrad_pending", [])
        for it in pend:
            it[3] += 1
        if group:
            d["wgrad_group"] = []
            counts = [ops.gemm_group_tiles(*g[:6]) for g in group]
            if min(counts) > 0 and sum(counts) >= 96:
                pend.extend([g[:6], c, 0, 0] for g, c in zip(group, counts))
            else:
                global WGRAD_GROUP
                saved, WGRAD_GROUP = WGRAD_GROUP, False
                try:
                    with self._side():
                        for A, B_, out, Mo, No, Kr, slot in group:
                            self._wgrad(d, A, B_, out, Mo, No, Kr, slot=slot)
                finally:
                    WGRAD_GROUP = saved
        for parts in plan_group_launches(pend, final, WGRAD_CARRY):
            with self._side():
                ops.gemm_group_part(parts)
        jobs = d.get("slab_jobs")
        if jobs:
            with self._side():
                ops.reduce_slabs_multi(jobs)
            d["slab_jobs"] = []

    def _bias_grad(self, d, dy, Mrows, N, gname):
        ops.colsum_reduce(dy, d["cs_part"], self.P.g(self.n(gname)), Mrows, N)

    def _ln_job(self, part, nparts, C, wname, bname, resid_bias=None):
        ow, ob = self.P.off(self.n(wname)), self.P.off(self.n(bname))
        assert ob == ow + C
        if resid_bias is None:
            return (part, self.P.grad[ow:ow + 2 * C], nparts, 2 * C)
        return (part, self.P.grad[ow:ow + 2 * C], nparts, 3 * C, self.P.g(self.n(resid_bias)), 2 * C)

    def _ln_grads(self, d, nparts, C, wname, bname, resid_bias=None):
        ow, ob = self.P.off(self.n(wname)), self.P.off(self.n(bname))
        assert ob == ow + C
        if resid_bias is None:
            ops.colreduce_seg(d["ln_part"], self.P.grad[ow:ow + 2 * C], nparts, 2 * C)
        else:
            ops.colreduce_seg(d["ln_part"], self.P.grad[ow:ow + 2 * C], nparts, 3 * C, out2=self.P.g(self.n(resid_bias)), split=2 * C)

    def forward(self, x, training=True, refresh=True, step_seed=0):
        cfg, P = self.cfg, self.P
        B, L = x.shape
        p_res, p_attn, p_act, p_in = self.drop_probs(training)
        slots = []
        sseed = lambda layer, site: self.site_seed(step_seed, layer, site)
        recording = ops._rec() is not None
        if refresh:
            self.refresh_weights()
        d = self.bufs(B, L)
        C, E, H, Fd, K, G = cfg.conv_dim, cfg.embed, cfg.heads, cfg.ffn, cfg.pos_k, cfg.pos_groups
        D, Cg = E // H, E // G
        Ts, T, M, Tp = d["Ts"], d["T"], d["M"], d["Tp"]
        fe = "feature_extractor.conv_layers.%d."
        ops.conv0_fwd(x, self.b(fe % 0 + "0.weight"), self.b(fe % 0 + "0.bias"), self.b(fe % 0 + "2.1.weight"),
                      self.b(fe % 0 + "2.1.bias"), d["z"][0], B, L, C, cfg.conv_kernels[0], cfg.conv_strides[0], stats=d["conv0_stats"])
        for i in range(1, len(Ts)):
            k, s, Tin, Tout = cfg.conv_kernels[i], cfg.conv_strides[i], Ts[i - 1], Ts[i]
            ops.gemm(Op(d["z"][i - 1], s * C, rpb=Tout, rbstride=Tin * C), Op(self.wk[i], k * C), d["y"][i], B * Tout, C, k * C,
                     bias=self.b(fe % i + "0.bias"))
            ops.layernorm_fwd(d["y"][i], self.b(fe % i + "2.1.weight"), self.b(fe % i + "2.1.bias"), d["z"][i], None,
                              d["cmean"][i], d["crstd"][i], B * Tout, C, act=1)
        ops.layernorm_fwd(d["z"][-1], self.b("layer_norm.weight"), self.b("layer_norm.bias"), d["h0"], None, d["fmean"],
                          d["frstd"], M, C)
        dsc = ops.gemm(Op(d["h0"], C), self.W("post_extract_proj.weight", C), d["x0"], M, E, C, bias=self.b("post_extract_proj.bias"),
                       drop_p=p_in, drop_seed=sseed(-1, self.SITE_IN))
        if p_in > 0 and recording:
            self._slot(slots, dsc, None, -1, self.SITE_IN)
        ops.pad_rows(d["x0"], d["xpad"], B, T, E, T + K, K // 2)
        if POSCONV_MFMA and ops.posconv_supported(T, K, G, Cg):
            ops.posconv_mfma(d["xpad"], self.pos_wf, d["xin"][0], d["x0"], B, T, K, G, Cg, bias=self.b("encoder.pos_conv.0.bias"), c2=d["pc_pre"])
        else:
            ops.gemm(Op(d["xpad"], E, rpb=T, rbstride=(T + K) * E, cin=Cg, cout=E, bs2=Cg), Op(self.pos_wf, K * Cg, bs2=Cg * K * Cg),
                     d["xin"][0], M, Cg, K * Cg, nb2=G, ldc=E, c_bs2=Cg, bias=self.b("encoder.pos_conv.0.bias"), bias_bs2=Cg,
                     act=ACT_GELU, c2=d["pc_pre"], R=d["x0"], rmode=1)
        if p_res > 0:
# ... 264 lines not shown
                ops.gemm(Op(d["d_ctx"], E, bs1=T * E, bs2=D), Op(qkv, 3 * E, bs1=T * 3 * E, bs2=D, offset=2 * E), d["S"], T, T, D,
                         ldc=Tp, c_bs1=H * T * Tp, c_bs2=T * Tp, **bq)
                if p_attn > 0:
                    self._slot(slots, ops.dropout_rows(d["S"], d["S"], B * H * T, T, Tp, sseed(n, self.SITE_ATTN), p_attn), ops.DROPOUT_ROWS_SEED, n, self.SITE_ATTN)
                ops.softmax_bwd(Pn, d["S"], d["dS"], B * H * T, T, Tp, Tp)
                sc = D ** -0.5
                dS = Op(d["dS"], Tp, bs1=H * T * Tp, bs2=T * Tp)
                ops.gemm(dS, Op(qkv, 3 * E, bs1=T * 3 * E, bs2=D, offset=E), dqkv, T, D, T, b_t=True, alpha=sc, ldc=3 * E,
                         c_bs1=T * 3 * E, c_bs2=D, c_offset=0, **bq)
                ops.gemm(dS, Op(qkv, 3 * E, bs1=T * 3 * E, bs2=D, offset=0), dqkv, T, D, T, a_t=True, b_t=True, alpha=sc, ldc=3 * E,
                         c_bs1=T * 3 * E, c_bs2=D, c_offset=E, **bq)
            with self._side():
                if not (FUSED_BIAS_GRAD and d["fused_attn"]):
                    ops.colsum_reduce(dqkv, d["cs_part"], self._qkv_view(pn, "bias"), M, 3 * E)
                self._wgrad(d, Op(dqkv, 3 * E), Op(d["h1"][n], E), self._qkv_view(pn, "weight"), 3 * E, E, Mp, slot=3)
            ops.gemm(Op(dqkv, 3 * E), self.W(pn + "self_attn.q_proj.weight", E), d["d_h"], M, E, 3 * E, b_t=True)
            dout, lyr = mask3_of([m_ for m_ in active if m_ < n])
            e = ops.layernorm_bwd(d["d_h"], xin, d["m1"][n], d["r1"][n], self.b(pn + "self_attn_layer_norm.weight"), None, dx,
                                  other, otherb, d["ln_part2"] if BATCH_REDUCE else d["ln_part"], M, E, sum_dres=True,
                                  din=(sseed(n, self.SITE_1), p_res), dout=dout)
            if p_res > 0:
                self._slot(slots, e, ops.LN_BWD_DIN_SEED, n, self.SITE_1)
                if lyr is not None:
                    self._slot(slots, e, ops.LN_BWD_DOUT_SEED, lyr, self.SITE_3)
            if BATCH_REDUCE:
                jobs.append(self._ln_job(d["ln_part2"], nlnM, E, pn + "self_attn_layer_norm.weight", pn + "self_attn_layer_norm.bias",
                                         resid_bias=pn + "self_attn.out_proj.bias"))
                ops.colreduce_multi(jobs)
            else:
                self._ln_grads(d, nlnM, E, pn + "self_attn_layer_norm.weight", pn + "self_attn_layer_norm.bias",
                               resid_bias=pn + "self_attn.out_proj.bias")
            cur = (cur + 1) % NR
            (dx, dxb), (other, otherb) = rot[cur], rot[(cur + 1) % NR]
            self._flush_slabs(d, final=(n == active[0]))
            self._join_side()
            this_off = P.off(self.n(pn + "self_attn_layer_norm.weight"))
            ready_off = this_off if not d.get("wgrad_pending") else prev_off
            prev_off = this_off
            if self.on_grads_ready is not None and ready_off is not None:
                ops.host_callback(self.on_grads_ready, ready_off)
        pb = K // 2 - 1
        if p_res > 0:
            self._slot(slots, ops.dropout(dx, dx, None, M * E, sseed(-1, self.SITE_ENC), p_res), ops.DROPOUT_SEED, -1, self.SITE_ENC)
        ops.pad_rows(dx, d["dcpad"], B, T, E, T + K, pb, pre=d["pc_pre"], ract=ACT_GELU)
        ops.colsum_reduce(d["dcpad"], d["cs_part"], P.g(self.n("encoder.pos_conv.0.bias")), B * (T + K), E)
        dwf = d["dwf"]
        if POSCONV_MFMA and ops.posconv_wgrad_supported(T, K, G, Cg):
            ops.posconv_wgrad(d["dcpad"], pb, d["xpad"], dwf, B, T, K, G, Cg)
        else:
            self._wgrad(d, Op(d["dcpad"], E, rpb=T, rbstride=(T + K) * E, bs2=Cg, offset=pb * E),
                        Op(d["xpad"], E, rpb=T, rbstride=(T + K) * E, cin=Cg, cout=E, bs2=Cg), dwf, Cg, K * Cg, M,
                        nb2=G, c_bs2=Cg * K * Cg, ldc=K * Cg)
        ops.posconv_weight_bwd(dwf, self.b("encoder.pos_conv.0.weight_v"), self.b("encoder.pos_conv.0.weight_g"), self.pos_norm,
                               self.ws_small, P.g(self.n("encoder.pos_conv.0.weight_v")), P.g(self.n("encoder.pos_conv.0.weight_g")),
                               E, Cg, K)
        if POSCONV_MFMA and ops.posconv_supported(T, K, G, Cg):
            ops.posconv_mfma(d["dcpad"], self.pos_wd, other, dx, B, T, K, G, Cg)
        else:
            ops.gemm(Op(d["dcpad"], E, rpb=T, rbstride=(T + K) * E, cin=Cg, cout=E, bs2=Cg), Op(self.pos_wd, K * Cg, bs2=Cg * K * Cg),
                     other, M, Cg, K * Cg, nb2=G, ldc=E, c_bs2=Cg, R=dx, rmode=1)
        dx0 = other
        if p_in > 0:
            self._slot(slots, ops.dropout(dx0, dx0, otherb, M * E, sseed(-1, self.SITE_IN), p_in), ops.DROPOUT_SEED, -1, self.SITE_IN)
        else:
            ops.cast_bf16(dx0, otherb, M * E)
        self._bias_grad(d, dx0, M, E, "post_extract_proj.bias")
        self._wgrad(d, Op(otherb, E), Op(d["h0"], C), P.g(self.n("post_extract_proj.weight")), E, C, M)
        ops.gemm(Op(otherb, E), self.W("post_extract_proj.weight", C), d["d_h"], M, C, E, b_t=True)
        ops.layernorm_bwd(d["d_h"], d["z"][-1], d["fmean"], d["frstd"], self.b("layer_norm.weight"), None, None, None, d["dz"][-1],
                          d["ln_part"], M, C)
        self._ln_grads(d, nlnM, C, "layer_norm.weight", "layer_norm.bias")
        fe = "feature_extractor.conv_layers.%d."
        for i in reversed(range(1, len(Ts))):
            k, s, Tin, Tout = cfg.conv_kernels[i], cfg.conv_strides[i], Ts[i - 1], Ts[i]
            Mi = B * Tout
            Q, Rp = d["dyp_geom"][i]
            dyp = d["dyp"][i]
            ops.layernorm_bwd(d["dz"][i], d["y"][i], d["cmean"][i], d["crstd"][i], self.b(fe % i + "2.1.weight"),
                              self.b(fe % i + "2.1.bias"), None, None, dyp, d["ln_part"], Mi, C, act=1,
                              out_rpb=Tout, out_rbstride=Rp * C, out_off=Q * C, sum_dres=2)
            self._ln_grads(d, ops.layernorm_bwd_nparts(Mi), C, fe % i + "2.1.weight", fe % i + "2.1.bias", resid_bias=fe % i + "0.bias")
            dwk = d["dwk"][: C * k * C].view(C, k * C)
            self._wgrad(d, Op(dyp, C, rpb=Tout, rbstride=Rp * C, offset=Q * C), Op(d["z"][i - 1], s * C, rpb=Tout, rbstride=Tin * C), dwk,
                        C, k * C, Mi)
            ops.conv_weight_unpack_grad(dwk, P.g(self.n(fe % i + "0.weight")), C, C, k)
            blk = 0
            for p in range(s):
                nq = len(range(p, k, s))
                Up = (Tin - 1 - p) // s
                if nq == 0:
                    raise NotImplementedError("conv layer with kernel < stride")
                ops.gemm(Op(dyp, C, rpb=Up + 1, rbstride=Rp * C, offset=(Q - (nq - 1)) * C), Op(self.wd[i], C, offset=blk * C * C),
                         d["dz"][i - 1], B * (Up + 1), C, nq * C, b_t=True, ldc=s * C, c_rpb=Up + 1, c_rbstride=Tin * C, c_offset=p * C)
                blk += nq
        ops.conv0_bwd(x, self.b(fe % 0 + "0.weight"), self.b(fe % 0 + "0.bias"), self.b(fe % 0 + "2.1.weight"),
                      self.b(fe % 0 + "2.1.bias"), d["dz"][0], d["conv0_ws"], P.g(self.n(fe % 0 + "0.weight")),
                      P.g(self.n(fe % 0 + "0.bias")), P.g(self.n(fe % 0 + "2.1.weight")), P.g(self.n(fe % 0 + "2.1.bias")),
                      B, L, C, cfg.conv_kernels[0], cfg.conv_strides[0], stats=d["conv0_stats"])
        return slots

    def _qkv_view(self, pn, kind):
        E = self.cfg.embed
        o = self.P.off(self.n(pn + "self_attn.q_proj." + kind))
        n = 3 * E * E if kind == "weight" else 3 * E
        v = self.P.grad[o:o + n]
        return v.view(3 * E, E) if kind == "weight" else v
```

scl-deepfake-audio-detection_amd/lib.py:

```python
import ctypes
import os

import torch

HERE = os.path.dirname(os.path.abspath(__file__))
LIB_PATH = os.environ.get("SCL_LIB_PATH") or os.path.join(HERE, "libscl_hip.so")
FLAT = 0x7FFFFFFF

_lib = None


class SclError(RuntimeError):
    pass


class SclOperand(ctypes.Structure):
    _fields_ = [("ptr", ctypes.c_void_p), ("bs1", ctypes.c_int64), ("bs2", ctypes.c_int64),
                ("rbstride", ctypes.c_int64), ("cout", ctypes.c_int64), ("rpb", ctypes.c_int32),
                ("ld", ctypes.c_int32), ("cin", ctypes.c_int32), ("_pad", ctypes.c_int32)]


class SclReduceJob(ctypes.Structure):
    _fields_ = [("part", ctypes.c_void_p), ("out", ctypes.c_void_p), ("out2", ctypes.c_void_p), ("pstride", ctypes.c_int64),
                ("nparts", ctypes.c_int32), ("C", ctypes.c_int32), ("split", ctypes.c_int32), ("_pad", ctypes.c_int32)]
# ... 4 lines not shown
                ("nslabs", ctypes.c_int32), ("_pad", ctypes.c_int32)]


class SclRsGeom(ctypes.Structure):
    _fields_ = [("B", ctypes.c_int32), ("H", ctypes.c_int32), ("W", ctypes.c_int32), ("r_lo", ctypes.c_int32), ("r_hi", ctypes.c_int32),
                ("_pad", ctypes.c_int32)]


class SclRsPackJob(ctypes.Structure):
    _fields_ = [("w", ctypes.c_void_p), ("out", ctypes.c_void_p), ("Co", ctypes.c_int32), ("Ci", ctypes.c_int32), ("ntaps", ctypes.c_int32),
                ("CINp", ctypes.c_int32), ("COUTp", ctypes.c_int32), ("transposed", ctypes.c_int32), ("ld", ctypes.c_int32), ("_pad", ctypes.c_int32)]


class SclRsConv(ctypes.Structure):
    _fields_ = [(n, ctypes.c_void_p) for n in ("inp", "wpk", "bias", "addend", "out", "act_a", "y1", "bnstats", "acc", "ticket", "gamma", "beta",
                                              "run_mean", "run_var", "nbt", "stats_out", "dgamma", "dbeta")] + \
               [("nvalid", ctypes.c_double), ("geom", SclRsGeom), ("shift", ctypes.c_int32 * 6), ("cin", ctypes.c_int32), ("cout", ctypes.c_int32),
                ("ntaps", ctypes.c_int32), ("stat_mode", ctypes.c_int32), ("training", ctypes.c_int32), ("epi_act", ctypes.c_int32),
                ("eps", ctypes.c_float), ("momentum", ctypes.c_float)]


class SclBtseBio(ctypes.Structure):
    _fields_ = [("emb", ctypes.c_void_p), ("lw", (ctypes.c_void_p * 18) * 8), ("Ws", ctypes.c_void_p), ("bs", ctypes.c_void_p),
                ("bio", ctypes.c_void_p), ("lens", ctypes.c_void_p), ("ws", ctypes.c_void_p), ("out", ctypes.c_void_p),
                ("d_out", ctypes.c_void_p), ("slab", ctypes.c_void_p), ("ws_stride", ctypes.c_int64), ("slab_ld", ctypes.c_int64),
                ("go", (ctypes.c_int32 * 18) * 8), ("go_emb", ctypes.c_int32), ("go_Ws", ctypes.c_int32), ("go_bs", ctypes.c_int32)] + \
               [(n, ctypes.c_int32) for n in ("n_layers", "n_bios", "bio_out", "L", "B", "out_ld", "dout_ld", "bio_dim", "n_heads", "pf_dim", "window")]


class SclGemmDesc(ctypes.Structure):
    _fields_ = [("A", SclOperand), ("B", SclOperand), ("C", ctypes.c_void_p), ("C2", ctypes.c_void_p),
                ("R", ctypes.c_void_p), ("bias", ctypes.c_void_p),
                ("c_bs1", ctypes.c_int64), ("c_bs2", ctypes.c_int64), ("c_rbstride", ctypes.c_int64),
                ("c_split_stride", ctypes.c_int64), ("bias_bs2", ctypes.c_int64),
                ("c_rpb", ctypes.c_int32), ("ldc", ctypes.c_int32),
                ("M", ctypes.c_int32), ("N", ctypes.c_int32), ("K", ctypes.c_int32),
                ("nb1", ctypes.c_int32), ("nb2", ctypes.c_int32), ("splitk", ctypes.c_int32),
                ("flags", ctypes.c_int32), ("alpha", ctypes.c_float), ("drop_p", ctypes.c_float),
                ("drop_seed", ctypes.c_uint32), ("_pad", ctypes.c_int32), ("colsum_part", ctypes.c_void_p)]


GEMM_A_T, GEMM_B_T, GEMM_C_F32, GEMM_C2_F32, GEMM_R_F32 = 1, 2, 4, 8, 16
GEMM_HAS_BIAS, GEMM_HAS_C2, GEMM_DROPOUT = 0x20, 0x40, 0x80
GEMM_NO_DMA = 0x00100000
GEMM_NO_BIG = 0x00200000
GEMM_FORCE_BIG = 0x04000000
GEMM_NO_P8 = 0x00400000
GEMM_FORCE_P8 = 0x00800000
GEMM_NO_W8 = 0x01000000
GEMM_FORCE_W8 = 0x02000000
GEMM_FORCE_X2 = 0x08000000
GEMM_NO_X2 = 0x10000000
GEMM_AB_F32 = 0x40000000
GEMM_C_SPLIT3 = -0x80000000
GEMM_F32X3 = 0x20000000
ACT_SHIFT, RMODE_SHIFT, RACT_SHIFT = 8, 12, 16
ACT_NONE, ACT_GELU, ACT_RELU, ACT_LEAKY = 0, 1, 2, 3
ACT_GELU_DC2 = 5
RACT_STORED = 4
KID_GEMM = 0
KID_AUG = 1
KID_GEMM_F32 = 2

_vp, _i32, _i64, _f32, _f64, _u32 = (ctypes.c_void_p, ctypes.c_int32, ctypes.c_int64, ctypes.c_float,
                                     ctypes.c_double, ctypes.c_uint32)


def _protos():
    P = ctypes.POINTER
    return {
        "scl_version": ([], _i32),
        "scl_last_error": ([], ctypes.c_char_p),
        "scl_build_flags": ([], _i32),
        "scl_prof_enable": ([_i32, _i32], _i32),
        "scl_prof_reserve": ([_i32, _i32], _i32),
        "scl_prof_read": ([_i32, P(_i64), P(_f64), P(_f64)], _i32),
        "scl_prof_read_launches": ([_i32, _i32, P(ctypes.c_float), P(_i32), P(_i64)], _i32),
        "scl_gemm_bf16": ([P(SclGemmDesc), _vp], _i32),
        "scl_gemm_bf16_group_ok": ([P(SclGemmDesc), _i32], _i32),
        "scl_gemm_bf16_group": ([P(SclGemmDesc), _i32, _vp], _i32),
        "scl_gemm_bf16_group_tiles": ([P(SclGemmDesc)], _i32),
        "scl_gemm_bf16_group_part": ([P(SclGemmDesc), P(_i32), P(_i32), _i32, _vp], _i32),
        "scl_reduce_slabs_f32": ([_vp, _vp, _i64, _i32, _i64, _vp], _i32),
        "scl_posconv_supported": ([_i32, _i32, _i32, _i32], _i32),
        "scl_posconv_wgrad_supported": ([_i32, _i32, _i32, _i32], _i32),
        "scl_posconv_wgrad": ([_vp, _i32, _vp, _vp, _i32, _i32, _i32, _i32, _i32, _vp], _i32),
        "scl_posconv_mfma": ([_vp, _vp, _vp, _vp, _vp, _vp, _i32, _i32, _i32, _i32, _i32, _i32, _vp], _i32),
        "scl_debug_gemm_stamps": ([_vp, _i32], _i32),
        "scl_debug_gemm_persistent_launches": ([], ctypes.c_longlong),
        "scl_gemm_uses_wide_tiles": ([P(SclGemmDesc)], _i32),
        "scl_gemm_colsum_rows": ([P(SclGemmDesc)], _i32),
        "scl_bn_nslabs": ([_i32], _i32),
        "scl_bn_fwd": ([_vp, _i32, _i32, _vp, _vp, _vp, _vp, _vp, _i32, _f32, _f32, _i32, _vp, _vp, _vp, _vp, _vp, _i32, _i32, _i32, _i64, _i64,
                        _i64, _i64, _vp], _i32),
        "scl_bn_bwd": ([_vp, _vp, _vp, _vp, _vp, _vp, _i32, _i32, _i32, _i32, _vp, _vp, _vp, _vp, _vp, _i32, _vp], _i32),
        "scl_pad_nhwc_f32": ([_vp, _i64, _i32, _vp, _i32, _i32, _i32, _i64, _i64, _i64, _i64, _vp], _i32),
        "scl_conv_pack_weights": ([_vp, _vp, _vp, _i32, _i32, _i32, _i32, _i32, _i32, _vp], _i32),
        "scl_conv_wgrad_finish": ([_vp, _vp, _i32, _i32, _i32, _i32, _i32, _i32, _i32, _vp], _i32),
        "scl_maxpool3_fwd": ([_vp, _i64, _i64, _i64, _i32, _i32, _i32, _vp, _vp, _vp], _i32),
        "scl_maxpool3_bwd": ([_vp, _vp, _i32, _i32, _i32, _vp, _i64, _i64, _i64, _vp], _i32),
        "scl_avgpool_fwd": ([_vp, _i32, _i32, _i32, _vp, _vp], _i32),
        "scl_avgpool_bwd": ([_vp, _i32, _i32, _i32, _vp, _vp], _i32),
        "scl_layernorm_fwd": ([_vp, _i32, _vp, _vp, _vp, _vp, _vp, _vp, _i32, _i32, _i64, _i64, _f32, _i32, _vp], _i32),
        "scl_layernorm_bwd_nparts": ([_i32], _i32),
        "scl_layernorm_bwd": ([_vp, _i32, _vp, _i32, _vp, _vp, _vp, _vp, _vp, _vp, _vp, _vp, _i32, _i32, _i64, _i64,
                               _i64, _i32, _i32, _i32, _i64, _i64, _u32, _f32, _u32, _f32, _vp], _i32),
        "scl_colreduce_f32": ([_vp, _vp, _i32, _i32, _i64, _i32, _vp], _i32),
        "scl_colsum_nparts": ([_i32], _i32),
        "scl_colsum_reduce_nparts": ([_i32, _i32], _i32),
        "scl_colsum": ([_vp, _i32, _vp, _i32, _i32, _i64, _vp], _i32),
        "scl_colreduce_multi": ([P(SclReduceJob), _i32, _vp], _i32),
        "scl_reduce_slabs_multi": ([P(SclSlabJob), _i32, _vp], _i32),
        "scl_colreduce_seg_f32": ([_vp, _vp, _i32, _i32, _i64, _i32, _vp, _vp, _vp, _i32, _vp], _i32),
        "scl_colsum_reduce": ([_vp, _i32, _vp, _vp, _vp, _i32, _i32, _i64, _vp], _i32),
        "scl_cast_f32_bf16": ([_vp, _vp, _i64, _vp], _i32),
        "scl_split3_f32_bf16": ([_vp, _i64, _i32, _i64, _vp, _i32, _vp], _i32),
        "scl_add_f32": ([_vp, _vp, _vp, _vp, _i64, _vp], _i32),
        "scl_pad_rows_bf16": ([_vp, _i32, _vp, _vp, _i32, _i32, _i32, _i32, _i32, _i32, _vp], _i32),
        "scl_col2im_bf16": ([_vp, _vp, _i32, _i32, _i32, _i32, _i32, _i32, _vp], _i32),
        "scl_conv_weight_pack": ([_vp, _vp, _vp, _i32, _i32, _i32, _i32, _vp], _i32),
        "scl_conv_weight_unpack_grad": ([_vp, _vp, _i32, _i32, _i32, _vp], _i32),
        "scl_posconv_weight_pack": ([_vp, _vp, _vp, _vp, _vp, _i32, _i32, _i32, _vp], _i32),
        "scl_posconv_weight_bwd": ([_vp, _vp, _vp, _vp, _vp, _vp, _vp, _i32, _i32, _i32, _vp], _i32),
        "scl_dropout_f32": ([_vp, _vp, _vp, _i64, _u32, _f32, _vp], _i32),
        "scl_meanpool_fwd": ([_vp, _vp, _i32, _i32, _i32, _vp], _i32),
        "scl_meanpool_bwd": ([_vp, _vp, _vp, _i32, _i32, _i32, _i32, _f32, _u32, _vp], _i32),
        "scl_meanpool_fwd_f32": ([_vp, _vp, _i32, _i32, _i32, _vp], _i32),
        "scl_meanpool_bwd_f32": ([_vp, _vp, _vp, _i32, _i32, _i32, _i32, _f32, _u32, _vp], _i32),
        "scl_utt_head_fwd": ([_vp, _vp, _vp, _vp, _i32, _i32, _i32, _vp], _i32),
        "scl_utt_head_bwd": ([_vp, _vp, _vp, _vp, _vp, _vp, _vp, _vp, _vp, _i32, _i32, _i32, _vp], _i32),
        "scl_softmax_fwd": ([_vp, _vp, _i64, _i32, _i32, _i32, _vp], _i32),
        "scl_softmax_bwd": ([_vp, _vp, _vp, _i64, _i32, _i32, _i32, _vp], _i32),
        "scl_softmax_fwd_f32": ([_vp, _vp, _i64, _i32, _i32, _i32, _vp], _i32),
        "scl_attn_fwd": ([_vp, _vp, _vp, _i32, _i32, _i32, _i32, _f32, _f32, _u32, _vp], _i32),
        "scl_attn_fwd_fp8": ([_vp, _vp, _vp, _i32, _i32, _i32, _i32, _f32, _vp], _i32),
        "scl_attn_bwd": ([_vp, _vp, _vp, _vp, _vp, _vp, _i32, _i32, _i32, _i32, _f32, _f32, _u32, _vp], _i32),
        "scl_attn_fwd_long": ([_vp, _vp, _vp, _i32, _i32, _i32, _i32, _f32, _f32, _u32, _vp], _i32),
        "scl_attn_long_ws_bytes": ([_i32, _i32, _i32], _i64),
        "scl_attn_bwd_long": ([_vp, _vp, _vp, _vp, _vp, _vp, _i32, _i32, _i32, _i32, _f32, _f32, _u32, _vp], _i32),
        "scl_softmax_fwd_f32_long": ([_vp, _vp, _i64, _i32, _i32, _i32, _vp], _i32),
        "scl_conv0_fwd": ([_vp, _vp, _vp, _vp, _vp, _vp, _vp, _i32, _i32, _i32, _i32, _i32, _f32, _vp], _i32),
        "scl_conv0_fwd_f32": ([_vp, _vp, _vp, _vp, _vp, _vp, _i32, _i32, _i32, _i32, _i32, _f32, _vp], _i32),
        "scl_conv0_bwd_nparts": ([_i32, _i32, _i32, _i32], _i32),
        "scl_conv0_bwd": ([_vp, _vp, _vp, _vp, _vp, _vp, _vp, _vp, _vp, _vp, _vp, _vp, _i32, _i32, _i32, _i32, _i32, _f32, _vp], _i32),
        "scl_gat_score_nblocks": ([_i32], _i32),
        "scl_gat_score_fwd": ([_vp, _vp, _vp, _vp, _vp, _i32, _i32, _i32, _i32, _i32, _vp], _i32),
        "scl_gat_score_bwd": ([_vp, _vp, _vp, _vp, _vp, _vp, _vp, _vp, _i32, _i32, _i32, _i32, _i32, _vp], _i32),
        "scl_dropout_rows": ([_vp, _vp, _i64, _i32, _i32, _i32, _u32, _f32, _vp], _i32),
        "scl_rs_conv": ([P(SclRsConv), _vp], _i32),
        "scl_rs_pack_weights": ([P(SclRsPackJob), _i32, _vp], _i32),
        "scl_rs_wgrad_nslabs": ([_i32, _i32], _i32),
        "scl_rs_wgrad": ([_vp, _vp, _i32, _i32, _i32, P(_i32), P(SclRsGeom), _vp, _vp, _vp, _vp, _vp], _i32),
        "scl_rs_wgrad_reduce": ([_vp, _i32, _i32, _i32, _i32, _i32, _i32, _i32, _vp, _vp], _i32),
        "scl_rs_bn_act": ([_vp, _vp, _vp, _i32, _i32, P(SclRsGeom), _vp], _i32),
        "scl_rs_bn_bwd_apply": ([_vp, _vp, _vp, _vp, _i32, _i32, P(SclRsGeom), _vp], _i32),
        "scl_rs_attn_pool_fwd": ([_vp, _vp, _vp, _vp, _vp, _i32, P(SclRsGeom), _vp], _i32),
        "scl_rs_attn_pool_bwd": ([_vp, _vp, _vp, _vp, _vp, _vp, _i32, P(SclRsGeom), _vp], _i32),
        "scl_rs_bn_eval_stats": ([_vp, _vp, _vp, _vp, _f32, _i32, _vp, _vp], _i32),
        "scl_rs_copy": ([_vp, _vp, _i32, _i32, _i32, P(SclRsGeom), _vp], _i32),
        "scl_graph_post_fwd": ([_vp, _i32, _i32, _vp], _i32),
        "scl_graph_post_bwd": ([_vp, _i32, _i32, _vp], _i32),
        "scl_graph_pre_fwd": ([_vp, _i32, _i32, _vp], _i32),
        "scl_graph_pre_bwd": ([_vp, _i32, _i32, _vp], _i32),
        "scl_graph_drop": ([_vp, _vp, _i64, _u32, _vp, _vp, _i64, _u32, _f32, _vp], _i32),
        "scl_graph_drop_bwd": ([_vp, _vp, _vp, _i64, _u32, _vp, _vp, _vp, _i64, _u32, _f32, _vp], _i32),
        "scl_graph_final_fwd": ([_vp, _i32, _vp], _i32),
# ... 134 lines not shown
```

scl-deepfake-audio-detection_amd/ops.py:

```python
import ctypes
import os

import torch

from . import lib as L

FLAT = L.FLAT


def _stream():
    return ctypes.c_void_p(torch.cuda.current_stream().cuda_stream)


import threading

_TLS = threading.local()


def _rec():
    return getattr(_TLS, "rec", None)


def start_recording():
    _TLS.rec = []
# ... 131 lines not shown
    _call("scl_gemm_bf16_group_part", arr, t0, nt, n, _stream(), keep=(arr, t0, nt))


def gemm_colsum_rows(A, B, C, M, N, K, **kw):
    d = _gemm_desc(A, B, C, M, N, K, **kw)
    return L.load().scl_gemm_colsum_rows(ctypes.byref(d))


def gemm_wide_kind(A, B, C, M, N, K, **kw):
    d = _gemm_desc(A, B, C, M, N, K, **kw)
    return L.load().scl_gemm_uses_wide_tiles(ctypes.byref(d))


def _gemm_desc(A, B, C, M, N, K, *, a_t=False, b_t=False, bias=None, act=0, c2=None, R=None, rmode=0, ract=0,
               alpha=1.0, nb1=1, nb2=1, splitk=1, ldc=None, c_rpb=FLAT, c_rbstride=0, c_bs1=0, c_bs2=0,
               c_offset=0, bias_bs2=0, bias_offset=0, drop_p=0.0, drop_seed=0, c_split_stride=0, no_dma=False, no_big=False, no_p8=False,
               force_p8=False, force_big=False, no_w8=False, force_w8=False, force_x2=False, no_x2=False, colsum_part=None, x3=None):
    d = L.SclGemmDesc()
    d.A, d.B = A.c(), B.c()
    flags = 0
    assert A.t.dtype == B.t.dtype, "A and B must have the same element type"
    if A.t.dtype == torch.float32:
        flags |= L.GEMM_AB_F32
        if F32X3 if x3 is None else x3:
            flags |= L.GEMM_F32X3
    if a_t:
        flags |= L.GEMM_A_T
    if b_t:
        flags |= L.GEMM_B_T
    if C.dtype == torch.float32:
        flags |= L.GEMM_C_F32
    else:
        assert C.dtype == torch.bfloat16
    d.C = _ptr(C, c_offset)
    if c2 is not None:
        flags |= L.GEMM_HAS_C2
        if c2.dtype == torch.float32:
            flags |= L.GEMM_C2_F32
        d.C2 = _ptr(c2, c_offset)
    if R is not None:
        assert rmode in (1, 2)
        if R.dtype == torch.float32:
            flags |= L.GEMM_R_F32
        d.R = _ptr(R, c_offset)
    if bias is not None:
        assert bias.dtype == torch.float32
        flags |= L.GEMM_HAS_BIAS
        d.bias = _ptr(bias, bias_offset)
    if drop_p > 0.0:
        flags |= L.GEMM_DROPOUT
    if colsum_part is not None:
        assert colsum_part.dtype == torch.float32
        d.colsum_part = _ptr(colsum_part)
    if no_dma:
        flags |= L.GEMM_NO_DMA
    if no_big:
        flags |= L.GEMM_NO_BIG
    if force_big:
        flags |= L.GEMM_FORCE_BIG
    if no_p8:
        flags |= L.GEMM_NO_P8
    if force_p8:
        flags |= L.GEMM_FORCE_P8
    if no_w8:
        flags |= L.GEMM_NO_W8
    if force_w8:
        flags |= L.GEMM_FORCE_W8
    if force_x2:
        flags |= L.GEMM_FORCE_X2
    if no_x2:
        flags |= L.GEMM_NO_X2
    flags |= (act << L.ACT_SHIFT) | (rmode << L.RMODE_SHIFT) | (ract << L.RACT_SHIFT)
    d.c_bs1, d.c_bs2, d.c_rbstride, d.c_split_stride, d.bias_bs2 = c_bs1, c_bs2, c_rbstride, c_split_stride, bias_bs2
    d.c_rpb, d.ldc = c_rpb, (N if ldc is None else ldc)
    d.M, d.N, d.K, d.nb1, d.nb2, d.splitk = M, N, K, nb1, nb2, splitk
    d.flags, d.alpha, d.drop_p, d.drop_seed = flags, alpha, drop_p, drop_seed
    return d


def reduce_slabs(slabs, out, n, nslabs, stride):
    _call("scl_reduce_slabs_f32", _ptr(slabs), _ptr(out), n, nslabs, stride, _stream())


def prof_enable(kid, on):
    _call("scl_prof_enable", kid, 1 if on else 0)


def prof_reserve(kid, n_pairs):
    _call("scl_prof_reserve", kid, n_pairs)


def prof_read_launches(kid, cap=65536):
    n = ctypes.c_int64(0)
    _call("scl_prof_read_launches", kid, 0, None, None, ctypes.byref(n))
    k = min(int(n.value), cap)
    if k == 0:
        return []
    ms = (ctypes.c_float * k)()
    meta = (ctypes.c_int32 * (8 * k))()
    _call("scl_prof_read_launches", kid, k, ms, meta, ctypes.byref(n))
    return [(float(ms[i]), tuple(int(meta[8 * i + j]) for j in range(8))) for i in range(k)]


def prof_read(kid):
    n, ms, fl = ctypes.c_int64(0), ctypes.c_double(0), ctypes.c_double(0)
    _call("scl_prof_read", kid, ctypes.byref(n), ctypes.byref(ms), ctypes.byref(fl))
    return n.value, ms.value, fl.value


def _p(t, offset=0):
    return None if t is None else _ptr(t, offset)


def _isf32(t):
    return 1 if t.dtype == torch.float32 else 0


def layernorm_fwd(x, gamma, beta, y_bf16, y_f32, mean, rstd, M, C, act=0, ldx=None, ldy=None, eps=1e-5):
    _call("scl_layernorm_fwd", _p(x), _isf32(x), _p(gamma), _p(beta), _p(y_bf16), _p(y_f32), _p(mean), _p(rstd),
                                       M, C, ldx or C, ldy or C, eps, act, _stream())


def layernorm_bwd_nparts(M):
    return L.load().scl_layernorm_bwd_nparts(M)


LN_BWD_DIN_SEED, LN_BWD_DOUT_SEED = 22, 24
ATTN_FWD_SEED, ATTN_BWD_SEED, DROPOUT_SEED = 9, 12, 4
ATTN_FWD_LONG_SEED, ATTN_BWD_LONG_SEED = 9, 12


def layernorm_bwd(dy, x, mean, rstd, gamma, beta, dres, dx_f32, dx_bf16, part, M, C, act=0, sum_dres=False, out_rpb=0,
                  out_rbstride=0, out_off=0, din=(0, 0.0), dout=(0, 0.0)):
    return _call("scl_layernorm_bwd", _p(dy), _isf32(dy), _p(x), _isf32(x), _p(mean), _p(rstd), _p(gamma), _p(beta),
                 _p(dres), _p(dx_f32), _p(dx_bf16), _p(part), M, C, C, C, C, act, int(sum_dres), out_rpb, out_rbstride, out_off,
                 int(din[0]), float(din[1]), int(dout[0]), float(dout[1]), _stream())


def colreduce(part, out, nparts, C, pstride=None, accumulate=False):
    _call("scl_colreduce_f32", _p(part), _p(out), nparts, C, pstride or C, 1 if accumulate else 0, _stream())


def colreduce_multi(jobs):
    arr = (L.SclReduceJob * len(jobs))()
    for i, jb in enumerate(jobs):
        part, out, nparts, C = jb[:4]
        out2, split = (jb[4], jb[5]) if len(jb) > 4 and jb[4] is not None else (None, 0)
        arr[i].part, arr[i].out, arr[i].out2 = _p(part), _p(out), _p(out2)
        arr[i].pstride, arr[i].nparts, arr[i].C, arr[i].split = C, nparts, C, split
    _call("scl_colreduce_multi", arr, len(jobs), _stream(), keep=arr)


def colsum_nparts(M):
    return L.load().scl_colsum_nparts(M)


def colsum_reduce_nparts(M, N):
    return L.load().scl_colsum_reduce_nparts(M, N)


def colsum(x, part, M, N, ld=None):
    _call("scl_colsum", _p(x), _isf32(x), _p(part), M, N, ld or N, _stream())


_COUNTERS = {}

# ... 395 lines not shown
```

Before: 1664.

## Tile posconv pack/apply via LDS, fuse slab reduce with unpack, slab-major w8 grid

The posconv weight pack and weight-grad apply kernels now stage one output channel's tile in LDS, so global reads and writes are coalesced instead of strided scatter. The split-K slab reduction for conv weight grads now writes straight into the unpacked weight layout, removing a separate unpack pass. The w8 GEMM gets a slab-major flattened grid for transposed split-K launches. It also keeps the batched row-offset path enabled in w8s instead of falling back to mode 0, and caches column offsets. These touch several unrelated kernels; the larger LDS tiles can lower occupancy, and the new grid mapping changes how work is spread across XCDs.

Measured after the change: 1668 (median of 3 runs). No clear change (+0.2%).

```diff
diff --git a/include/scl_hip.h b/include/scl_hip.h
--- a/include/scl_hip.h
+++ b/include/scl_hip.h
@@ -105,6 +105,7 @@
 int scl_gemm_splitk_finish(const SclGemmDesc* desc, const float* slabs, int nslabs, int64_t stride, void* stream);
 
 int scl_reduce_slabs_f32(const float* slabs, float* out, int64_t n, int nslabs, int64_t stride, void* stream);
+int scl_reduce_slabs_unpack_f32(const float* slabs, float* dw, int Co, int Ci, int k, int nslabs, int64_t stride, void* stream);
 #define SCL_SLAB_MAX_JOBS 8
 typedef struct SclSlabJob {
     const float* slabs;
diff --git a/scl-deepfake-audio-detection_amd/csrc/elementwise.hip b/scl-deepfake-audio-detection_amd/csrc/elementwise.hip
--- a/scl-deepfake-audio-detection_amd/csrc/elementwise.hip
+++ b/scl-deepfake-audio-detection_amd/csrc/elementwise.hip
@@ -172,17 +172,36 @@
         out[threadIdx.x] = do_sqrt ? sqrtf(t) : t;
     }
 }
-__global__ void posconv_pack_kernel(const float* __restrict__ v, const float* __restrict__ g, const float* __restrict__ norm,
-                                    bf16_t* __restrict__ wf, bf16_t* __restrict__ wd, int E, int Cg, int K) {
-    const int64_t n = (int64_t)E * Cg * K;
-    for (int64_t i = (int64_t)blockIdx.x * blockDim.x + threadIdx.x; i < n; i += (int64_t)gridDim.x * blockDim.x) {
-        const int j = (int)(i % K);
-        const int ci = (int)((i / K) % Cg);
-        const int cot = (int)(i / ((int64_t)Cg * K));
-        const int grp = cot / Cg, co = cot % Cg;
+__global__ __launch_bounds__(256) void posconv_pack_kernel(const float* __restrict__ v, const float* __restrict__ g, const float* __restrict__ norm,
+                                                           bf16_t* __restrict__ wf, bf16_t* __restrict__ wd, int E, int Cg, int K, int pairs) {
+    extern __shared__ bf16_t pk_tile[];
+    const int P = (Cg + 2) & ~1;
+    const bool second = (int)blockIdx.x >= E;
+    const int b = second ? (int)blockIdx.x - E : (int)blockIdx.x;
+    const int grp = b / Cg, c = b - grp * Cg;
+    const int64_t src0 = second ? ((int64_t)grp * Cg * Cg + c) * K : (int64_t)b * Cg * K;
+    const int64_t rstride = second ? (int64_t)Cg * K : K;
+    const int n = Cg * K;
+#pragma unroll 4
+    for (int e = threadIdx.x; e < n; e += blockDim.x) {
+        const int r = e / K, j = e - r * K;
+        const int64_t i = src0 + r * rstride + j;
         const bf16_t val = f2bf(g[j] * v[i] / norm[j]);
-        wf[(((int64_t)grp * Cg + co) * K + j) * Cg + ci] = val;
-        wd[(((int64_t)grp * Cg + ci) * K + (K - 1 - j)) * Cg + co] = val;
+        pk_tile[(second ? K - 1 - j : j) * P + r] = val;
+    }
+    __syncthreads();
+    bf16_t* out = (second ? wd : wf) + (int64_t)b * n;
+    if (pairs) {
+        const int h = Cg >> 1;
+        for (int e = threadIdx.x; e < K * h; e += blockDim.x) {
+            const int row = e / h, cp = e - row * h;
+            reinterpret_cast<unsigned*>(out)[e] = *reinterpret_cast<const unsigned*>(pk_tile + row * P + 2 * cp);
+        }
+    } else {
+        for (int e = threadIdx.x; e < n; e += blockDim.x) {
+            const int row = e / Cg;
+            out[e] = pk_tile[row * P + (e - row * Cg)];
+        }
     }
 }
 __global__ __launch_bounds__(256) void posconv_wbwd_dot_part_kernel(const float* __restrict__ dwf, const float* __restrict__ v,
@@ -210,16 +229,23 @@
         part[(int64_t)cot * K + threadIdx.x] = t;
     }
 }
-__global__ void posconv_wbwd_apply_kernel(const float* __restrict__ dwf, const float* __restrict__ v, const float* __restrict__ g,
-                                          const float* __restrict__ norm, const float* __restrict__ sdot,
-                                          float* __restrict__ dv, float* __restrict__ dg, int E, int Cg, int K) {
-    const int64_t n = (int64_t)E * Cg * K;
-    for (int64_t i = (int64_t)blockIdx.x * blockDim.x + threadIdx.x; i < n; i += (int64_t)gridDim.x * blockDim.x) {
-        const int j = (int)(i % K);
-        const int ci = (int)((i / K) % Cg);
-        const int cot = (int)(i / ((int64_t)Cg * K));
-        const int grp = cot / Cg, co = cot % Cg;
-        const float dw = dwf[(((int64_t)grp * Cg + co) * K + j) * Cg + ci];
+__global__ __launch_bounds__(256) void posconv_wbwd_apply_kernel(const float* __restrict__ dwf, const float* __restrict__ v, const float* __restrict__ g,
+                                                                 const float* __restrict__ norm, const float* __restrict__ sdot,
+                                                                 float* __restrict__ dv, float* __restrict__ dg, int E, int Cg, int K) {
+    extern __shared__ float ap_tile[];
+    const int cot = blockIdx.x, n = Cg * K;
+    const float* db = dwf + (int64_t)cot * n;
+#pragma unroll 4
+    for (int e = threadIdx.x; e < n; e += blockDim.x) {
+        const int j = e / Cg;
+        ap_tile[j * (Cg + 1) + (e - j * Cg)] = db[e];
+    }
+    __syncthreads();
+#pragma unroll 4
+    for (int e = threadIdx.x; e < n; e += blockDim.x) {
+        const int ci = e / K, j = e - ci * K;
+        const int64_t i = (int64_t)cot * n + e;
+        const float dw = ap_tile[j * (Cg + 1) + ci];
         const float nj = norm[j];
         dv[i] = g[j] / nj * dw - g[j] * sdot[j] / (nj * nj * nj) * v[i];
         if (i < K) dg[i] = sdot[i] / norm[i];
@@ -378,7 +404,10 @@
         hipLaunchKernelGGL(posconv_norm_part_kernel, dim3((nrows + rpb - 1) / rpb), dim3(256), 0, s, v, part, nrows, K, rpb);
         hipLaunchKernelGGL(posconv_vec_finish_kernel, dim3(1), dim3(1024 / K * K), 0, s, part, norm, (nrows + rpb - 1) / rpb, K, 1);
     }
-    hipLaunchKernelGGL(posconv_pack_kernel, dim3(grid_for((int64_t)E * Cg * K)), dim3(256), 0, s, v, g, norm, (bf16_t*)wf, (bf16_t*)wd, E, Cg, K);
+    const size_t lds = (size_t)K * ((Cg + 2) & ~1) * sizeof(bf16_t);
+    SCL_REQUIRE(lds <= 64 * 1024, "posconv_weight_pack: Cg*K too large for the LDS tile");
+    const int pairs = !(Cg & 1) && !(((uintptr_t)wf | (uintptr_t)wd) & 3);
+    hipLaunchKernelGGL(posconv_pack_kernel, dim3(2 * E), dim3(256), lds, s, v, g, norm, (bf16_t*)wf, (bf16_t*)wd, E, Cg, K, pairs);
     return scl_check_launch("scl_posconv_weight_pack");
 }
 extern "C" int scl_posconv_weight_bwd(const float* dwf, const float* v, const float* g, const float* norm, float* sdot_ws,
@@ -398,7 +427,13 @@
         hipLaunchKernelGGL(posconv_wbwd_dot_part_kernel, dim3(E), dim3(256), lds, s, dwf, v, part, Cg, K);
         hipLaunchKernelGGL(posconv_vec_finish_kernel, dim3(1), dim3(1024 / K * K), 0, s, part, sdot_ws, E, K, 0);
     }
-    hipLaunchKernelGGL(posconv_wbwd_apply_kernel, dim3(grid_for((int64_t)E * Cg * K)), dim3(256), 0, s, dwf, v, g, norm, sdot_ws, dv, dg, E, Cg, K);
+    const size_t lds_ap = (size_t)K * (Cg + 1) * sizeof(float);
+    static bool ap_attr_set = false;
+    if (!ap_attr_set) {
+        hipFuncSetAttribute((const void*)posconv_wbwd_apply_kernel, hipFuncAttributeMaxDynamicSharedMemorySize, 160 * 1024);
+        ap_attr_set = true;
+    }
+    hipLaunchKernelGGL(posconv_wbwd_apply_kernel, dim3(E), dim3(256), lds_ap, s, dwf, v, g, norm, sdot_ws, dv, dg, E, Cg, K);
     return scl_check_launch("scl_posconv_weight_bwd");
 }
 
diff --git a/scl-deepfake-audio-detection_amd/csrc/gemm.hip b/scl-deepfake-audio-detection_amd/csrc/gemm.hip
--- a/scl-deepfake-audio-detection_amd/csrc/gemm.hip
+++ b/scl-deepfake-audio-detection_amd/csrc/gemm.hip
@@ -655,6 +655,24 @@
                 out[j] = s;
             }
         }
+    }
+}
+
+__global__ void scl_reduce_slabs_unpack_kernel(const float* __restrict__ slabs, float* __restrict__ dw, int Co, int Ci, int k,
+                                               int nslabs, int64_t stride) {
+    const int64_t n = (int64_t)Co * k * Ci;
+    const int64_t i0 = ((int64_t)blockIdx.x * blockDim.x + threadIdx.x) * 4;
+    const int64_t step = (int64_t)gridDim.x * blockDim.x * 4;
+    for (int64_t i = i0; i < n; i += step) {
+        float4 s = *reinterpret_cast<const float4*>(slabs + i);
+        for (int q = 1; q < nslabs; ++q) {
+            const float4 t = *reinterpret_cast<const float4*>(slabs + q * stride + i);
+            s.x += t.x; s.y += t.y; s.z += t.z; s.w += t.w;
+        }
+        const int64_t row = i / Ci;
+        const int ci = (int)(i - row * Ci), co = (int)(row / k), j = (int)(row - (int64_t)co * k);
+        float* o = dw + ((int64_t)co * Ci + ci) * k + j;
+        o[0] = s.x; o[k] = s.y; o[2 * k] = s.z; o[3 * k] = s.w;
     }
 }
 
@@ -1064,3 +1082,12 @@
     hipLaunchKernelGGL(scl_reduce_slabs_kernel, dim3(blocks), dim3(256), 0, (hipStream_t)stream, slabs, out, n, nslabs, stride);
     return scl_check_launch("scl_reduce_slabs_f32");
 }
+
+extern "C" int scl_reduce_slabs_unpack_f32(const float* slabs, float* dw, int Co, int Ci, int k, int nslabs, int64_t stride, void* stream) {
+    SCL_REQUIRE(slabs && dw && Co > 0 && Ci > 0 && k > 0 && nslabs >= 1, "reduce_slabs_unpack: bad args");
+    SCL_REQUIRE(((uintptr_t)slabs & 15) == 0 && (stride & 3) == 0 && (Ci & 3) == 0, "reduce_slabs_unpack: alignment");
+    const int64_t n = (int64_t)Co * k * Ci;
+    int blocks = (int)((n / 4 + 255) / 256); if (blocks > 2048) blocks = 2048; if (blocks < 1) blocks = 1;
+    hipLaunchKernelGGL(scl_reduce_slabs_unpack_kernel, dim3(blocks), dim3(256), 0, (hipStream_t)stream, slabs, dw, Co, Ci, k, nslabs, stride);
+    return scl_check_launch("scl_reduce_slabs_unpack_f32");
+}
diff --git a/scl-deepfake-audio-detection_amd/csrc/gemm_w8.hip b/scl-deepfake-audio-detection_amd/csrc/gemm_w8.hip
--- a/scl-deepfake-audio-detection_amd/csrc/gemm_w8.hip
+++ b/scl-deepfake-audio-detection_amd/csrc/gemm_w8.hip
@@ -52,12 +52,11 @@
 struct W8T {
     __amdgpu_buffer_rsrc_t rsrc;
     unsigned voff[4];
-    int col0_, collimit_;
+    unsigned coff[2];
     bool batched;
     __device__ __forceinline__ void set_batched(bool b) { batched = b; }
     __device__ __forceinline__ void init(const OpK& o, const char* base, int col0, int collimit, int lane, int wave) {
         rsrc = make_rsrc(base);
-        col0_ = col0; collimit_ = collimit;
         const int s16 = lane & 15;
 #pragma unroll
         for (int i = 0; i < 4; ++i) {
@@ -65,20 +64,15 @@
             const int kr = 4 * (p & 15) + (lane >> 4);
             const int sw = (kr & 3) | (((kr >> 3) & 1) << 2);
             const int col = col0 + (p >> 4) * 128 + 8 * ((((s16 >> 1) ^ sw) << 1) | (s16 & 1));
-            voff[i] = col < collimit ? (unsigned)kr * o.ld_bytes + col_off(o, (unsigned)col) : OOB;
+            if (!(i & 1)) coff[i >> 1] = col < collimit ? col_off(o, (unsigned)col) : OOB;
+            voff[i] = col < collimit ? (unsigned)kr * o.ld_bytes + coff[i >> 1] : OOB;
         }
     }
     __device__ __forceinline__ void rows(const OpK& o, int krow, int lane, int wave) {
         if (!batched) return;
-        const int s16 = lane & 15;
-#pragma unroll
-        for (int i = 0; i < 4; ++i) {
-            const int p = wave * 4 + i;
-            const int kr = 4 * (p & 15) + (lane >> 4);
-            const int sw = (kr & 3) | (((kr >> 3) & 1) << 2);
-            const int col = col0_ + (p >> 4) * 128 + 8 * ((((s16 >> 1) ^ sw) << 1) | (s16 & 1));
-            voff[i] = col < collimit_ ? row_off(o, (unsigned)(krow + kr)) + col_off(o, (unsigned)col) : OOB;
-        }
+        const int kr0 = krow + 4 * ((wave * 4) & 15) + (lane >> 4);
+#pragma unroll
+        for (int i = 0; i < 4; ++i) voff[i] = coff[i >> 1] != OOB ? row_off(o, (unsigned)(kr0 + 4 * i)) + coff[i >> 1] : OOB;
     }
     template <int I0>
     __device__ __forceinline__ void issue2(char* img, int wave, unsigned soff, bool live) const {
@@ -102,6 +96,19 @@
 __device__ __forceinline__ bf16x8 w8_frag(const char* img, int gb, int ks, int lane) {
     if (T) return frag_t_raw(img + (gb >> 3) * TILE_BYTES, gb & 7, ks, lane);
     return frag_k(img, gb, ks, lane);
+}
+
+__device__ __forceinline__ bool w8_slab_major(const GemmK& d, int& bid, int& nblk, int& bz) {
+    if (!(d.debug & 32)) return true;
+    const int tiles = ((d.M + d.tile_m - 1) / d.tile_m) * ((d.N + W8_BN - 1) / W8_BN);
+    const int total = tiles * d.splitk;
+    const int x = bid & 7, idx = bid >> 3, q = total >> 3, r = total & 7;
+    const int s = (x < r ? x * (q + 1) : r * (q + 1) + (x - r) * q) + idx;
+    if (s >= total) return false;
+    bz = __builtin_amdgcn_readfirstlane(s / tiles);
+    bid = __builtin_amdgcn_readfirstlane(s - bz * tiles);
+    nblk = tiles;
+    return true;
 }
 
 #define W8_MFMA_PHASE(MH, NH, FBSEL, NI)                                                                   \
@@ -206,10 +213,11 @@
     w8_stamp(d, 0, lane, wave);
     const int tiles_m = (d.M + d.tile_m - 1) / d.tile_m, tiles_n = (d.N + W8_BN - 1) / W8_BN;
     int tm, tn;
-    tile_coords(blockIdx.x, gridDim.x, tiles_m, tiles_n, tm, tn, d.group_m);
+    int bid = blockIdx.x, nblk = gridDim.x, z = blockIdx.z;
+    if (!w8_slab_major(d, bid, nblk, z)) return;
+    tile_coords(bid, nblk, tiles_m, tiles_n, tm, tn, d.group_m);
     const int m0 = tm * d.tile_m, n0 = tn * W8_BN;
     const int mlimit = min(d.M, m0 + d.tile_m);
-    int z = blockIdx.z;
     const int ksplit = __builtin_amdgcn_readfirstlane(z % d.splitk); z /= d.splitk;
     const int z1 = __builtin_amdgcn_readfirstlane(z / d.nb2), z2 = z - z1 * d.nb2;
     const int nk_total = d.K / BK;
@@ -301,10 +309,10 @@
 };
 
 template <bool AT, bool BT, int RBW>
-__device__ __forceinline__ void w8s_body(const GemmK& d, char* smem, const typename W8Sel<AT>::type& la, const typename W8Sel<BT>::type& lb,
+__device__ __forceinline__ void w8s_body(const GemmK& d, char* smem, typename W8Sel<AT>::type& la, typename W8Sel<BT>::type& lb,
                                          int nk, unsigned soffA, unsigned soffB, int ab, int m0, int n0, int mlimit,
-                                         int z1, int z2, int ksplit, int lane, int wave, int wc) {
-    const unsigned stepA = W8Sel<AT>::type::kstep(d.A), stepB = W8Sel<BT>::type::kstep(d.B);
+                                         int z1, int z2, int ksplit, int lane, int wave, int wc, int krow0) {
+    const unsigned stepA = la.step(d.A), stepB = lb.step(d.B);
     f32x4 acc[RBW][4];
 #pragma unroll
     for (int i = 0; i < RBW; ++i)
@@ -335,6 +343,7 @@
         const bool live2b = live2;
 #endif
         soffA += stepA; soffB += stepB;
+        la.rows(d.A, krow0 + (kt + 2) * BK, lane, wave);
 #define W8S_Q_FIRST(j, R0, R1)                                                                                               \
         RD::template go<R0, R1, false>(fa1, fb1, a_cur, tB, ab, nbk, 1, lane);                                               \
         __builtin_amdgcn_sched_barrier(0);                                                                                   \
@@ -353,6 +362,7 @@
         __builtin_amdgcn_s_barrier();
         __builtin_amdgcn_sched_barrier(0);
         const char* tBn = bimg + ((kt & 1) ^ 1) * W8_OPB;
+        lb.rows(d.B, krow0 + (kt + 2) * BK, lane, wave);
 #define W8S_B_ISSUE(j) if ((j) < 2) { lb.issue1(tB, wave, soffB, live2b, 2 * (j)); lb.issue1(tB, wave, soffB, live2b, 2 * (j) + 1); }
 #define W8S_Q_SECOND(j, R0, R1)                                                                                              \
         RD::template go<R0, R1, false>(fa0, fb0, a_nxt, tBn, ab, nbk, 0, lane);                                              \
@@ -403,7 +413,7 @@
     }
 }
 
-template <bool AT, bool BT, int RB0, int RB1, bool SEQ = false>
+template <bool AT, bool BT, int RB0, int RB1, bool SEQ = false, bool ROWS = true>
 __device__ __forceinline__ void w8s_tile(const GemmK& d, char* smem, const int bid, const int nblk, const int bz) {
     const int tid = threadIdx.x, lane = tid & 63;
     const int wave = __builtin_amdgcn_readfirstlane(tid >> 6);
@@ -433,30 +443,36 @@
     typename W8Sel<BT>::type lb;
     la.init(d.A, Ab, m0, mlimit, lane, wave);
     lb.init(d.B, Bb, n0, d.N, lane, wave);
-    la.set_batched(false); lb.set_batched(false);
-    const unsigned stepA = W8Sel<AT>::type::kstep(d.A), stepB = W8Sel<BT>::type::kstep(d.B);
+    la.set_batched(ROWS && AT && (d.debug & 4));
+    lb.set_batched(ROWS && BT && (d.debug & 8));
+    const unsigned stepA = la.step(d.A), stepB = lb.step(d.B);
     unsigned soffA = (unsigned)kt0 * stepA, soffB = (unsigned)kt0 * stepB;
+    const int krow0 = kt0 * BK;
+    la.rows(d.A, krow0, lane, wave); lb.rows(d.B, krow0, lane, wave);
     la.template issue2<0>(smem, wave, soffA, nk > 0); la.template issue2<2>(smem, wave, soffA, nk > 0);
     lb.template issue2<0>(smem + W8_NA * W8_OPB, wave, soffB, nk > 0); lb.template issue2<2>(smem + W8_NA * W8_OPB, wave, soffB, nk > 0);
     soffA += stepA; soffB += stepB;
+    la.rows(d.A, krow0 + BK, lane, wave); lb.rows(d.B, krow0 + BK, lane, wave);
     la.template issue2<0>(smem + W8_OPB, wave, soffA, nk > 1); la.template issue2<2>(smem + W8_OPB, wave, soffA, nk > 1);
     lb.template issue2<0>(smem + (W8_NA + 1) * W8_OPB, wave, soffB, nk > 1); lb.template issue2<2>(smem + (W8_NA + 1) * W8_OPB, wave, soffB, nk > 1);
     asm volatile("s_waitcnt vmcnt(8)" ::: "memory");
     w8_stamp(d, 1, lane, wave);
     __builtin_amdgcn_s_barrier();
     if (RB0 == RB1) {
-        w8s_body<AT, BT, RB0>(d, smem, la, lb, nk, soffA, soffB, wr * RB0, m0, n0, mlimit, z1, z2, ksplit, lane, wave, wc);
+        w8s_body<AT, BT, RB0>(d, smem, la, lb, nk, soffA, soffB, wr * RB0, m0, n0, mlimit, z1, z2, ksplit, lane, wave, wc, krow0);
     } else if (wr == 0) {
-        w8s_body<AT, BT, RB0>(d, smem, la, lb, nk, soffA, soffB, 0, m0, n0, mlimit, z1, z2, ksplit, lane, wave, wc);
+        w8s_body<AT, BT, RB0>(d, smem, la, lb, nk, soffA, soffB, 0, m0, n0, mlimit, z1, z2, ksplit, lane, wave, wc, krow0);
     } else {
-        w8s_body<AT, BT, RB1>(d, smem, la, lb, nk, soffA, soffB, RB0, m0, n0, mlimit, z1, z2, ksplit, lane, wave, wc);
+        w8s_body<AT, BT, RB1>(d, smem, la, lb, nk, soffA, soffB, RB0, m0, n0, mlimit, z1, z2, ksplit, lane, wave, wc, krow0);
     }
 }
 
 template <bool AT, bool BT, int RB0, int RB1>
 __global__ __launch_bounds__(512, 2) void scl_gemm_w8s_kernel(const GemmK d) {
     extern __shared__ __attribute__((aligned(16))) char smem[];
-    w8s_tile<AT, BT, RB0, RB1>(d, smem, blockIdx.x, gridDim.x, blockIdx.z);
+    int bid = blockIdx.x, nblk = gridDim.x, bz = blockIdx.z;
+    if (!w8_slab_major(d, bid, nblk, bz)) return;
+    w8s_tile<AT, BT, RB0, RB1>(d, smem, bid, nblk, bz);
 }
 
 struct GemmGroupK {
@@ -485,9 +501,9 @@
     mem = __builtin_amdgcn_readfirstlane(mem);
     const int t = __builtin_amdgcn_readfirstlane(pos - gp->first[mem] + gp->tile0[mem]);
 #ifdef SCL_EXPERIMENTS
-    if (!g.xcd_major) { w8s_tile<AT, BT, RB0, RB1, false>(*(const GemmK*)&gp->k[mem], smem, t, gp->ntiles[mem], 0); return; }
-#endif
-    w8s_tile<AT, BT, RB0, RB1, true>(*(const GemmK*)&gp->k[mem], smem, t, gp->ntiles[mem], 0);
+    if (!g.xcd_major) { w8s_tile<AT, BT, RB0, RB1, false, false>(*(const GemmK*)&gp->k[mem], smem, t, gp->ntiles[mem], 0); return; }
+#endif
+    w8s_tile<AT, BT, RB0, RB1, true, false>(*(const GemmK*)&gp->k[mem], smem, t, gp->ntiles[mem], 0);
 }
 
 #ifdef SCL_EXPERIMENTS
@@ -794,14 +810,18 @@
     const char* me = getenv("SCL_W8_MODE");
     int mode = (me && *me) ? atoi(me) : 1;
     if (at && bt) {
-        if ((long long)k.A.rpb < (long long)k.K) { k.debug |= 4; mode = 0; }
-        if ((long long)k.B.rpb < (long long)k.K) { k.debug |= 8; mode = 0; }
+        if ((long long)k.A.rpb < (long long)k.K) k.debug |= 4;
+        if ((long long)k.B.rpb < (long long)k.K) k.debug |= 8;
     }
     {
         static const bool epi_generic = [] { const char* e = getenv("SCL_W8_EPI_GENERIC"); return e && atoi(e) != 0; }();
         if (epi_generic) k.debug |= 16;
     }
     dim3 g = grid;
+    if (at && bt && k.splitk > 1 && zdim == (long long)k.splitk && k.nb2 == 1 && !(k.flags & SCL_GEMM_STAMPS)) {
+        k.debug |= 32;
+        g = dim3((unsigned)(plan.tiles * zdim), 1, 1);
+    }
 #ifdef SCL_EXPERIMENTS
     {
         const char* sg = getenv("SCL_W8_STAGGER");
diff --git a/scl-deepfake-audio-detection_amd/encoder.py b/scl-deepfake-audio-detection_amd/encoder.py
--- a/scl-deepfake-audio-detection_amd/encoder.py
+++ b/scl-deepfake-audio-detection_amd/encoder.py
@@ -274,7 +274,7 @@
         if self.wstream is not None:
             ops.stream_wait(torch.cuda.current_stream(), self.wstream)
 
-    def _wgrad(self, d, A, B_, out, Mo, No, Kr, slot=None, **kw):
+    def _wgrad(self, d, A, B_, out, Mo, No, Kr, slot=None, unpack=None, **kw):
         ksteps = (Kr + 63) // 64
         if WGRAD_GROUP and slot is not None and not kw and Kr % 64 == 0 and ksteps >= WGRAD_GROUP_MIN_KSTEPS:
             d.setdefault("wgrad_group", []).append((A, B_, out, Mo, No, Kr, slot))
@@ -288,6 +288,8 @@
                 sk = skw
         if sk == 1:
             ops.gemm(A, B_, out, Mo, No, Kr, a_t=True, b_t=True, **kw)
+            if unpack is not None:
+                ops.conv_weight_unpack_grad(out, *unpack)
             return
         n = out.numel()
         if BATCH_SLABS and slot is not None:
@@ -302,7 +304,12 @@
             d.setdefault("slabs_keep", []).append(d["slab"])
             d["slab"] = torch.empty(sk * n, dtype=torch.float32, device=self.dev)
         ops.gemm(A, B_, d["slab"], Mo, No, Kr, a_t=True, b_t=True, splitk=sk, c_split_stride=n, **kw)
+        if unpack is not None and unpack[2] % 4 == 0:
+            ops.reduce_slabs_unpack(d["slab"], unpack[0], unpack[1], unpack[2], unpack[3], sk, n)
+            return
         ops.reduce_slabs(d["slab"], out, n, sk, n)
+        if unpack is not None:
+            ops.conv_weight_unpack_grad(out, *unpack)
 
     def _flush_slabs(self, d, final=True):
         group = d.get("wgrad_group")
@@ -733,8 +740,7 @@
             self._ln_grads(d, ops.layernorm_bwd_nparts(Mi), C, fe % i + "2.1.weight", fe % i + "2.1.bias", resid_bias=fe % i + "0.bias")
             dwk = d["dwk"][: C * k * C].view(C, k * C)
             self._wgrad(d, Op(dyp, C, rpb=Tout, rbstride=Rp * C, offset=Q * C), Op(d["z"][i - 1], s * C, rpb=Tout, rbstride=Tin * C), dwk,
-                        C, k * C, Mi)
-            ops.conv_weight_unpack_grad(dwk, P.g(self.n(fe % i + "0.weight")), C, C, k)
+                        C, k * C, Mi, unpack=(P.g(self.n(fe % i + "0.weight")), C, C, k))
             blk = 0
             for p in range(s):
                 nq = len(range(p, k, s))
diff --git a/scl-deepfake-audio-detection_amd/lib.py b/scl-deepfake-audio-detection_amd/lib.py
--- a/scl-deepfake-audio-detection_amd/lib.py
+++ b/scl-deepfake-audio-detection_amd/lib.py
@@ -110,6 +110,7 @@
         "scl_gemm_bf16_group_tiles": ([P(SclGemmDesc)], _i32),
         "scl_gemm_bf16_group_part": ([P(SclGemmDesc), P(_i32), P(_i32), _i32, _vp], _i32),
         "scl_reduce_slabs_f32": ([_vp, _vp, _i64, _i32, _i64, _vp], _i32),
+        "scl_reduce_slabs_unpack_f32": ([_vp, _vp, _i32, _i32, _i32, _i32, _i64, _vp], _i32),
         "scl_posconv_supported": ([_i32, _i32, _i32, _i32], _i32),
         "scl_posconv_wgrad_supported": ([_i32, _i32, _i32, _i32], _i32),
         "scl_posconv_wgrad": ([_vp, _i32, _vp, _vp, _i32, _i32, _i32, _i32, _i32, _vp], _i32),
diff --git a/scl-deepfake-audio-detection_amd/ops.py b/scl-deepfake-audio-detection_amd/ops.py
--- a/scl-deepfake-audio-detection_amd/ops.py
+++ b/scl-deepfake-audio-detection_amd/ops.py
@@ -237,6 +237,10 @@
     _call("scl_reduce_slabs_f32", _ptr(slabs), _ptr(out), n, nslabs, stride, _stream())
 
 
+def reduce_slabs_unpack(slabs, dw, Co, Ci, k, nslabs, stride):
+    _call("scl_reduce_slabs_unpack_f32", _ptr(slabs), _ptr(dw), Co, Ci, k, nslabs, stride, _stream())
+
+
 def prof_enable(kid, on):
     _call("scl_prof_enable", kid, 1 if on else 0)
 
```
